# agstub/shakti-fenics

Hardware: NVIDIA B200
Metric: time_steps_per_sec_at_16M_dofs (higher is better)
Workload: dtype f64

## Files before the change

shakti-fenics_b200/csrc/amg.cu:

```cuda
#include "amg.h"
#include "comm.h"

#include <algorithm>
#include <cstdlib>
#include <cmath>
#include <map>
#include <numeric>

namespace shakti {


static int aggregate(const HostCsr& A, int32_t n, const std::vector<uint8_t>& excl, const std::vector<uint8_t>& strong,
                     std::vector<int32_t>& agg) {
  agg.assign(n, -1);
  std::vector<uint8_t> free_(n, 1);
  for (int32_t i = 0; i < n; ++i)
    if (!excl.empty() && excl[i]) free_[i] = 0;
  int32_t na = 0;
  auto nb = [&](int32_t i, auto&& f) {
    for (int32_t k = A.rowptr[i]; k < A.rowptr[i + 1]; ++k) {
      const int32_t j = A.col[k];
      if (j < n && j != i && (excl.empty() || !excl[j]) && (strong.empty() || strong[k])) f(j);
    }
  };
  for (int32_t i = 0; i < n; ++i) {
    if (!free_[i]) continue;
    bool ok = true;
    nb(i, [&](int32_t j) { ok &= (free_[j] != 0); });
    if (!ok) continue;
    agg[i] = na;
    free_[i] = 0;
    nb(i, [&](int32_t j) { agg[j] = na; free_[j] = 0; });
    ++na;
  }
  {
    std::vector<int32_t> snap(agg);
    std::vector<int32_t> size(na, 0);
    for (int32_t i = 0; i < n; ++i)
      if (snap[i] >= 0) size[snap[i]]++;
    for (int32_t i = 0; i < n; ++i) {
      if (!free_[i]) continue;
      int32_t best = -1;
      nb(i, [&](int32_t j) {
        if (snap[j] >= 0 && (best < 0 || size[snap[j]] < size[best])) best = snap[j];
      });
      if (best >= 0) { agg[i] = best; size[best]++; free_[i] = 0; }
    }
  }
  for (int32_t i = 0; i < n; ++i) {
    if (!free_[i]) continue;
    agg[i] = na;
    free_[i] = 0;
    nb(i, [&](int32_t j) { if (free_[j]) { agg[j] = na; free_[j] = 0; } });
    ++na;
  }
  return na;
}

static HostCsr product_pattern(const HostCsr& A, const HostCsr& B) {
  HostCsr C;
  C.n_rows = A.n_rows;
  C.n_cols = B.n_cols;
  C.rowptr.assign(A.n_rows + 1, 0);
  std::vector<int32_t> mark(B.n_cols, -1), tmp;
  for (int64_t i = 0; i < A.n_rows; ++i) {
    tmp.clear();
    for (int32_t k = A.rowptr[i]; k < A.rowptr[i + 1]; ++k) {
      const int32_t j = A.col[k];
      if (j >= B.n_rows) continue;
      for (int32_t l = B.rowptr[j]; l < B.rowptr[j + 1]; ++l) {
        const int32_t c = B.col[l];
        if (mark[c] != (int32_t)i) { mark[c] = (int32_t)i; tmp.push_back(c); }
      }
    }
    std::sort(tmp.begin(), tmp.end());
    C.col.insert(C.col.end(), tmp.begin(), tmp.end());
    if (C.col.size() > 2000000000ULL) throw Error(SHAKTI_ERR_INVALID, "AMG product pattern too large");
    C.rowptr[i + 1] = (int32_t)C.col.size();
  }
  return C;
}


__global__ void amg_dinv_kernel(int32_t n, const int32_t* __restrict__ diag_pos, const double* __restrict__ val,
                                double* __restrict__ dinv) {
  const int32_t i = blockIdx.x * blockDim.x + threadIdx.x;
  if (i >= n) return;
  const double d = val[diag_pos[i]];
  dinv[i] = d != 0.0 ? 1.0 / d : 0.0;
}

__global__ void __launch_bounds__(256)
amg_prolongator_kernel(SellView A, const uint8_t* __restrict__ pmap, const int32_t* __restrict__ diag_pos,
                       const double* __restrict__ dinv, double omega, const int32_t* __restrict__ Pslice,
                       double* __restrict__ Pval) {
  const int32_t row = blockIdx.x * blockDim.x + threadIdx.x;
  if (row >= A.n_rows) return;
  const int32_t slice = row >> 5, lane = row & 31;
  const int32_t base = A.slice_ptr[slice];
  const int32_t w = (A.slice_ptr[slice + 1] - base) >> 5;
  const int32_t pbase = Pslice[slice] + lane;
  const int32_t dpos = diag_pos[row];
  const double s = omega * dinv[row];
  for (int k = 0; k < w; ++k) {
    const int32_t p = base + 32 * k + lane;
    const uint8_t t = pmap[p];
    if (t == 255) continue;
    const double v = (p == dpos ? 1.0 : 0.0) - s * A.val[p];
    Pval[pbase + 32 * (int32_t)t] += v;
  }
}

__global__ void amg_gather_vals_kernel(int64_t n, const int32_t* __restrict__ map, const double* __restrict__ src,
                                       double* __restrict__ out) {
  const int64_t stride = (int64_t)gridDim.x * blockDim.x;
  for (int64_t i = (int64_t)blockIdx.x * blockDim.x + threadIdx.x; i < n; i += stride) {
    const int32_t m = map[i];
    out[i] = m >= 0 ? src[m] : 0.0;
  }
}

__global__ void __launch_bounds__(128)
amg_spgemm_kernel(SellView A, const int32_t* __restrict__ Alen, SellView B, const int32_t* __restrict__ Blen,
                  int32_t Bn_rows, const int32_t* __restrict__ Cslice, const int32_t* __restrict__ Ccol,
                  const int32_t* __restrict__ Clen, double* __restrict__ Cval) {
  const int32_t row = blockIdx.x * blockDim.x + threadIdx.x;
  if (row >= A.n_rows) return;
  const int32_t lane = row & 31;
  const int32_t abase = A.slice_ptr[row >> 5] + lane;
  const int32_t cbase = Cslice[row >> 5] + lane;
  const int32_t clen = Clen[row];
  const int32_t alen = Alen[row];
  for (int ka = 0; ka < alen; ++ka) {
    const int32_t j = A.col[abase + 32 * ka];
    if (j >= Bn_rows) continue;
    const double a = A.val[abase + 32 * ka];
    if (a == 0.0) continue;
    const int32_t bbase = B.slice_ptr[j >> 5] + (j & 31);
    const int32_t blen = Blen[j];
    for (int kb = 0; kb < blen; ++kb) {
      const int32_t c = B.col[bbase + 32 * kb];
      const double b = B.val[bbase + 32 * kb];
      int lo = 0, hi = clen - 1;
      while (lo < hi) {
        const int mid = (lo + hi) >> 1;
        if (Ccol[cbase + 32 * mid] < c) lo = mid + 1; else hi = mid;
      }
      Cval[cbase + 32 * lo] += a * b;
    }
  }
}

__global__ void __launch_bounds__(128)
amg_spgemm_warp_kernel(SellView A, const int32_t* __restrict__ Alen, SellView B, const int32_t* __restrict__ Blen,
                       int32_t Bn_rows, const int32_t* __restrict__ Cslice, const int32_t* __restrict__ Ccol,
                       const int32_t* __restrict__ Clen, double* __restrict__ Cval) {
  const int32_t row = (blockIdx.x * blockDim.x + threadIdx.x) >> 5;
  const int lane = threadIdx.x & 31;
  if (row >= A.n_rows) return;
  const int32_t abase = A.slice_ptr[row >> 5] + (row & 31);
  const int32_t cbase = Cslice[row >> 5] + (row & 31);
  const int32_t clen = Clen[row], alen = Alen[row];
  for (int pos = lane; pos < clen; pos += 32) {
    const int32_t c = Ccol[cbase + 32 * pos];
    double acc = 0.0;
    for (int ka = 0; ka < alen; ++ka) {
      const int32_t j = A.col[abase + 32 * ka];
      if (j >= Bn_rows) continue;
      const double a = A.val[abase + 32 * ka];
      if (a == 0.0) continue;
      const int32_t bbase = B.slice_ptr[j >> 5] + (j & 31);
      int lo = 0, hi = Blen[j] - 1;
      while (lo < hi) {
        const int mid = (lo + hi) >> 1;
        if (B.col[bbase + 32 * mid] < c) lo = mid + 1; else hi = mid;
      }
      if (hi >= 0 && lo == hi && B.col[bbase + 32 * lo] == c) acc += a * B.val[bbase + 32 * lo];
    }
    Cval[cbase + 32 * pos] = acc;
  }
}

struct SpgemmPlan {
  bool built = false, ok = false;
  DevBuf<int64_t> prod_ptr;
  DevBuf<uint8_t> slot;
};

__global__ void __launch_bounds__(128)
amg_spgemm_count_kernel(SellView A, const int32_t* __restrict__ Alen, const int32_t* __restrict__ Blen, int32_t Bn_rows,
                        int32_t* __restrict__ slice_width) {
  const int32_t row = blockIdx.x * blockDim.x + threadIdx.x;
  int32_t cnt = 0;
  if (row < A.n_rows) {
    const int32_t abase = A.slice_ptr[row >> 5] + (row & 31);
    const int32_t alen = Alen[row];
    for (int ka = 0; ka < alen; ++ka) {
      const int32_t j = A.col[abase + 32 * ka];
      if (j < Bn_rows) cnt += Blen[j];
    }
  }
#pragma unroll
  for (int o = 16; o > 0; o >>= 1) cnt = max(cnt, __shfl_xor_sync(0xffffffffu, cnt, o));
  if ((threadIdx.x & 31) == 0 && (row >> 5) < A.n_slices) slice_width[row >> 5] = cnt;
}

__global__ void __launch_bounds__(128)
amg_spgemm_slots_kernel(SellView A, const int32_t* __restrict__ Alen, SellView B, const int32_t* __restrict__ Blen,
                        int32_t Bn_rows, const int32_t* __restrict__ Cslice, const int32_t* __restrict__ Ccol,
                        const int32_t* __restrict__ Clen, const int64_t* __restrict__ prod_ptr, uint8_t* __restrict__ slot) {
  const int32_t row = blockIdx.x * blockDim.x + threadIdx.x;
  if (row >= A.n_rows) return;
  const int32_t lane = row & 31;
  const int32_t abase = A.slice_ptr[row >> 5] + lane;
  const int32_t cbase = Cslice[row >> 5] + lane;
  const int32_t clen = Clen[row], alen = Alen[row];
  uint8_t* __restrict__ sp = slot + prod_ptr[row >> 5] + lane;
  int64_t t = 0;
  for (int ka = 0; ka < alen; ++ka) {
    const int32_t j = A.col[abase + 32 * ka];
    if (j >= Bn_rows) continue;
    const int32_t bbase = B.slice_ptr[j >> 5] + (j & 31);
    const int32_t blen = Blen[j];
    for (int kb = 0; kb < blen; ++kb, ++t) {
      const int32_t c = B.col[bbase + 32 * kb];
      int lo = 0, hi = clen - 1;
      while (lo < hi) {
        const int mid = (lo + hi) >> 1;
        if (Ccol[cbase + 32 * mid] < c) lo = mid + 1; else hi = mid;
      }
      sp[32 * t] = (uint8_t)lo;
    }
  }
}

__global__ void __launch_bounds__(128)
amg_spgemm_table_kernel(SellView A, const int32_t* __restrict__ Alen, SellView B, const int32_t* __restrict__ Blen,
                        int32_t Bn_rows, const int32_t* __restrict__ Cslice, const int32_t* __restrict__ Clen,
                        const int64_t* __restrict__ prod_ptr, const uint8_t* __restrict__ slot, double* __restrict__ Cval) {
  extern __shared__ double acc[];
  const int32_t row = blockIdx.x * blockDim.x + threadIdx.x;
  if (row >= A.n_rows) return;
  const int32_t lane = row & 31;
  const int32_t abase = A.slice_ptr[row >> 5] + lane;
  const int32_t clen = Clen[row], alen = Alen[row];
  double* __restrict__ my = acc + threadIdx.x;
  for (int k = 0; k < clen; ++k) my[k * 128] = 0.0;
  const uint8_t* __restrict__ sp = slot + prod_ptr[row >> 5] + lane;
  int64_t t = 0;
  for (int ka = 0; ka < alen; ++ka) {
    const int32_t j = A.col[abase + 32 * ka];
    if (j >= Bn_rows) continue;
    const double a = A.val[abase + 32 * ka];
    const int32_t bbase = B.slice_ptr[j >> 5] + (j & 31);
    const int32_t blen = Blen[j];
    for (int kb = 0; kb < blen; ++kb, ++t) my[(int)sp[32 * t] * 128] += a * B.val[bbase + 32 * kb];
  }
  double* __restrict__ cp = Cval + Cslice[row >> 5] + lane;
  for (int k = 0; k < clen; ++k) cp[32 * k] = my[k * 128];
}

static void build_spgemm_plan(const DevSell& A, const DevSell& B, const DevSell& C, SpgemmPlan& plan, cudaStream_t s) {
  plan.built = true;
  plan.ok = false;
  const size_t smem = (size_t)C.max_width * 128 * sizeof(double);
  if (A.n_rows == 0 || C.max_width > 255 || smem > 96 * 1024) return;
  DevBuf<int32_t> width;
  width.alloc_zero(A.n_slices, s);
  SHAKTI_LAUNCH(amg_spgemm_count_kernel, div_up((int64_t)A.n_slices * 32, 128), 128, 0, s, view(A), A.rowlen.p, B.rowlen.p, B.n_rows,
                width.p);
  const std::vector<int32_t> w = width.download(s);
  std::vector<int64_t> ptr(w.size() + 1, 0);
  for (size_t i = 0; i < w.size(); ++i) ptr[i + 1] = ptr[i] + 32 * (int64_t)w[i];
  plan.prod_ptr.upload(ptr);
  plan.slot.alloc((size_t)std::max<int64_t>(ptr.back(), 1));
  SHAKTI_LAUNCH(amg_spgemm_slots_kernel, div_up(A.n_rows, 128), 128, 0, s, view(A), A.rowlen.p, view(B), B.rowlen.p, B.n_rows,
                C.slice_ptr.p, C.col.p, C.rowlen.p, plan.prod_ptr.p, plan.slot.p);
  if (smem > 48 * 1024)
    SHAKTI_CUDA(cudaFuncSetAttribute(amg_spgemm_table_kernel, cudaFuncAttributeMaxDynamicSharedMemorySize, 96 * 1024));
  plan.ok = true;
}

static void spgemm_numeric(const DevSell& A, const DevSell& B, DevSell& C, SpgemmPlan& plan, cudaStream_t s) {
  if (A.n_rows == 0) return;
  if (A.n_rows <= 400000) {
    SHAKTI_LAUNCH(amg_spgemm_warp_kernel, div_up((int64_t)A.n_rows * 32, 128), 128, 0, s, view(A), A.rowlen.p, view(B), B.rowlen.p,
                  B.n_rows, C.slice_ptr.p, C.col.p, C.rowlen.p, C.val.p);
    return;
  }
  if (!plan.built) build_spgemm_plan(A, B, C, plan, s);
  if (plan.ok) {
    SHAKTI_LAUNCH(amg_spgemm_table_kernel, div_up(A.n_rows, 128), 128, (size_t)C.max_width * 128 * sizeof(double), s, view(A),
                  A.rowlen.p, view(B), B.rowlen.p, B.n_rows, C.slice_ptr.p, C.rowlen.p, plan.prod_ptr.p, plan.slot.p, C.val.p);
  } else {
    SHAKTI_CUDA(cudaMemsetAsync(C.val.p, 0, sizeof(double) * C.padded, s));
    SHAKTI_LAUNCH(amg_spgemm_kernel, div_up(A.n_rows, 128), 128, 0, s, view(A), A.rowlen.p, view(B), B.rowlen.p, B.n_rows,
                  C.slice_ptr.p, C.col.p, C.rowlen.p, C.val.p);
  }
}

__global__ void amg_dense_fill_kernel(SellView A, const int32_t* __restrict__ Alen, int32_t n, double* __restrict__ D) {
  const int32_t row = blockIdx.x * blockDim.x + threadIdx.x;
  if (row >= n) return;
  const int32_t base = A.slice_ptr[row >> 5] + (row & 31);
  for (int k = 0; k < Alen[row]; ++k) {
    const int32_t j = A.col[base + 32 * k];
    if (j < n) D[(size_t)row * 2 * n + j] += A.val[base + 32 * k];
  }
  D[(size_t)row * 2 * n + n + row] = 1.0;
}

__global__ void __launch_bounds__(1024)
amg_dense_invert_kernel(int32_t n, double* __restrict__ D, int* __restrict__ info) {
  extern __shared__ double fcol[];
  __shared__ int piv;
  __shared__ double pval;
  const int ld = 2 * n;
  for (int k = 0; k < n; ++k) {
    if (threadIdx.x < 32) {
      int p = k;
      double best = -1.0;
      for (int i = k + (int)threadIdx.x; i < n; i += 32) {
        const double v = fabs(D[(size_t)i * ld + k]);
        if (v > best) { best = v; p = i; }
      }
#pragma unroll
      for (int o = 16; o > 0; o >>= 1) {
        const double ob = __shfl_xor_sync(0xffffffffu, best, o);
        const int op = __shfl_xor_sync(0xffffffffu, p, o);
        if (ob > best || (ob == best && op < p)) { best = ob; p = op; }
      }
      if (threadIdx.x == 0) {
        piv = p;
        pval = D[(size_t)p * ld + k];
        if (!(best > 0.0)) *info = k + 1;
      }
    }
    __syncthreads();
    const int p = piv;
    const double inv = pval != 0.0 ? 1.0 / pval : 0.0;
    for (int j = threadIdx.x; j < ld; j += blockDim.x) {
      const double a = D[(size_t)p * ld + j], b = D[(size_t)k * ld + j];
      D[(size_t)p * ld + j] = b;
      D[(size_t)k * ld + j] = a * inv;
    }
    __syncthreads();
    for (int i = threadIdx.x; i < n; i += blockDim.x) fcol[i] = (i == k) ? 0.0 : D[(size_t)i * ld + k];
    __syncthreads();
    for (int idx = threadIdx.x; idx < n * ld; idx += blockDim.x) {
      const int i = idx / ld, j = idx - i * ld;
      const double f = fcol[i];
      if (f != 0.0) D[(size_t)i * ld + j] -= f * D[(size_t)k * ld + j];
    }
    __syncthreads();
  }
}

template <class TB, class TX>
__global__ void amg_dense_apply_kernel(int32_t n, const double* __restrict__ D, const TB* __restrict__ b,
                                       TX* __restrict__ x) {
  pdl_sync();
  const int warp = (blockIdx.x * blockDim.x + threadIdx.x) >> 5, lane = threadIdx.x & 31;
  if (warp >= n) return;
  const double* row = D + (size_t)warp * 2 * n + n;
  double acc = 0.0;
  for (int j = lane; j < n; j += 32) acc += row[j] * (double)b[j];
#pragma unroll
  for (int o = 16; o > 0; o >>= 1) acc += __shfl_xor_sync(0xffffffffu, acc, o);
  if (lane == 0) x[warp] = (TX)acc;
}

template <class T, int KG>
__global__ void __launch_bounds__(256)
amg_cheby_kernel(SellViewT<T> A, const T* __restrict__ dinv, const T* __restrict__ b, const T* __restrict__ x,
                 T* __restrict__ d, T* __restrict__ x_out, T c1, T c2) {
  pdl_sync();
  int32_t row;
  T acc = 0;
  if (KG == 1) {
    row = blockIdx.x * blockDim.x + threadIdx.x;
    const int32_t slice = row >> 5;
    if (slice >= A.n_slices) return;
    const int32_t base = A.slice_ptr[slice];
    const int32_t w = (A.slice_ptr[slice + 1] - base) >> 5;
    const int32_t* __restrict__ cp = A.col + base + (row & 31);
    const T* __restrict__ vp = A.val + base + (row & 31);
#pragma unroll 4
    for (int k = 0; k < w; ++k) acc += vp[32 * k] * x[cp[32 * k]];
  } else {
    __shared__ T psum[KG][32];
    const int32_t slice = blockIdx.x;
    const int lane = threadIdx.x & 31, g = threadIdx.x >> 5;
    row = slice * 32 + lane;
    const int32_t base = A.slice_ptr[slice];
    const int32_t w = (A.slice_ptr[slice + 1] - base) >> 5;
    const int32_t* __restrict__ cp = A.col + base + lane;
    const T* __restrict__ vp = A.val + base + lane;
    for (int k = g; k < w; k += KG) acc += vp[32 * k] * x[cp[32 * k]];
    psum[g][lane] = acc;
    __syncthreads();
    if (g != 0) return;
#pragma unroll
    for (int j = 1; j < KG; ++j) acc += psum[j][lane];
  }
  if (row >= A.n_rows) return;
  const T r = dinv[row] * (b[row] - acc);
  const T dn = c1 * d[row] + c2 * r;
  d[row] = dn;
  x_out[row] = x[row] + dn;
}
constexpr int32_t kChebyWideRowsBelow = 300000;
template <class T>
static void launch_cheby(SellViewT<T> A, const T* dinv, const T* b, const T* x, T* d, T* x_out, double c1, double c2, cudaStream_t s) {
  if (A.n_rows < kChebyWideRowsBelow)
    SHAKTI_LAUNCH_PDL((amg_cheby_kernel<T, 8>), A.n_slices, 256, 0, s, A, dinv, b, x, d, x_out, (T)c1, (T)c2);
  else
    SHAKTI_LAUNCH_PDL((amg_cheby_kernel<T, 1>), div_up((int64_t)A.n_slices * 32, 256), 256, 0, s, A, dinv, b, x, d, x_out, (T)c1, (T)c2);
}

__global__ void __launch_bounds__(256)
amg_cheby_h_kernel(int32_t n_rows, int32_t n_slices, const int32_t* __restrict__ slice_ptr, const int32_t* __restrict__ col,
                   const __half* __restrict__ val, const float* __restrict__ dinv, const float* __restrict__ b,
                   const float* __restrict__ x, float* __restrict__ d, float* __restrict__ x_out, float c1, float c2) {
  pdl_sync();
  const int32_t row = blockIdx.x * blockDim.x + threadIdx.x;
  const int32_t slice = row >> 5;
  if (slice >= n_slices) return;
  const int32_t base = slice_ptr[slice];
  const int32_t w = (slice_ptr[slice + 1] - base) >> 5;
  const int32_t* __restrict__ cp = col + base + (row & 31);
  const __half* __restrict__ vp = val + base + (row & 31);
  float acc = 0.f;
#pragma unroll 4
  for (int k = 0; k < w; ++k) acc += __half2float(vp[32 * k]) * x[cp[32 * k]];
  if (row >= n_rows) return;
  const float r = dinv[row] * b[row] - acc;
  const float dn = c1 * d[row] + c2 * r;
  d[row] = dn;
  x_out[row] = x[row] + dn;
}
__global__ void __launch_bounds__(256)
amg_resid_h_kernel(int32_t n_rows, int32_t n_slices, const int32_t* __restrict__ slice_ptr, const int32_t* __restrict__ col,
                   const __half* __restrict__ val, const float* __restrict__ dinv, const float* __restrict__ b,
                   const float* __restrict__ x, float* __restrict__ r) {
  pdl_sync();
  const int32_t row = blockIdx.x * blockDim.x + threadIdx.x;
  const int32_t slice = row >> 5;
  if (slice >= n_slices) return;
  const int32_t base = slice_ptr[slice];
  const int32_t w = (slice_ptr[slice + 1] - base) >> 5;
  const int32_t* __restrict__ cp = col + base + (row & 31);
  const __half* __restrict__ vp = val + base + (row & 31);
  float acc = 0.f;
#pragma unroll 4
  for (int k = 0; k < w; ++k) acc += __half2float(vp[32 * k]) * x[cp[32 * k]];
  if (row >= n_rows) return;
  const float di = dinv[row];
  r[row] = b[row] - (di != 0.f ? acc / di : 0.f);
}
static bool uses_half(const Amg::Impl& I, const DevSell& A);

template <class T>
__global__ void amg_cheby_first_kernel(int32_t n, const T* __restrict__ dinv, const T* __restrict__ b, T inv_theta,
                                       T* __restrict__ d, T* __restrict__ x) {
  pdl_sync();
  const int32_t i = blockIdx.x * blockDim.x + threadIdx.x;
  if (i >= n) return;
  const T v = dinv[i] * b[i] * inv_theta;
  d[i] = v;
  x[i] = v;
}

__global__ void __launch_bounds__(256)
amg_gershgorin_kernel(SellView A, const double* __restrict__ dinv, unsigned long long* __restrict__ out) {
  const int32_t row = blockIdx.x * blockDim.x + threadIdx.x;
  double v = 0.0;
  if (row < A.n_rows) {
    const int32_t base = A.slice_ptr[row >> 5] + (row & 31);
    const int32_t w = (A.slice_ptr[(row >> 5) + 1] - A.slice_ptr[row >> 5]) >> 5;
    double acc = 0.0;
    for (int k = 0; k < w; ++k) acc += fabs(A.val[base + 32 * k]);
    v = fabs(dinv[row]) * acc;
  }
#pragma unroll
  for (int o = 16; o > 0; o >>= 1) v = fmax(v, __shfl_xor_sync(0xffffffffu, v, o));
  if ((threadIdx.x & 31) == 0 && v > 0.0) atomicMax(out, (unsigned long long)__double_as_longlong(v));
}

__global__ void amg_pack_rows_kernel(int64_t n, const int32_t* __restrict__ pos, const double* __restrict__ val,
                                     double* __restrict__ out) {
  const int64_t i = (int64_t)blockIdx.x * blockDim.x + threadIdx.x;
  if (i >= n) return;
  const int32_t p = pos[i];
  out[i] = p >= 0 ? val[p] : 0.0;
}
__global__ void amg_unpack_rows_kernel(int64_t n, const int32_t* __restrict__ pos, const double* __restrict__ in,
                                       double* __restrict__ val) {
  const int64_t i = (int64_t)blockIdx.x * blockDim.x + threadIdx.x;
  if (i >= n) return;
  const int32_t p = pos[i];
  if (p >= 0) val[p] = in[i];
}
__global__ void amg_dense_rows_kernel(SellView A, const int32_t* __restrict__ Alen, const int32_t* __restrict__ colmap,
                                      int32_t n, int32_t N, double* __restrict__ D) {
  const int32_t row = blockIdx.x * blockDim.x + threadIdx.x;
  if (row >= n) return;
  const int32_t base = A.slice_ptr[row >> 5] + (row & 31);
  for (int k = 0; k < Alen[row]; ++k) D[(size_t)row * N + colmap[A.col[base + 32 * k]]] += A.val[base + 32 * k];
}
__global__ void amg_dense_assemble_kernel(int32_t N, int32_t nmax, int32_t nranks, const int32_t* __restrict__ off,
                                          const double* __restrict__ G, double* __restrict__ D) {
  const int64_t t = (int64_t)blockIdx.x * blockDim.x + threadIdx.x;
  if (t >= (int64_t)N * N) return;
  const int32_t gi = (int32_t)(t / N), j = (int32_t)(t - (int64_t)gi * N);
  int r = 0;
  while (r + 1 < nranks && off[r + 1] <= gi) ++r;
  const int32_t li = gi - off[r];
  D[(size_t)gi * 2 * N + j] = G[((size_t)r * nmax + li) * N + j];
  if (j == 0) D[(size_t)gi * 2 * N + N + gi] = 1.0;
}
template <class TO>
__global__ void amg_compact_kernel(int32_t N, int32_t nmax, int32_t nranks, const int32_t* __restrict__ off,
                                   const double* __restrict__ G, TO* __restrict__ out) {
  const int32_t gi = blockIdx.x * blockDim.x + threadIdx.x;
  if (gi >= N) return;
  int r = 0;
  while (r + 1 < nranks && off[r + 1] <= gi) ++r;
  out[gi] = (TO)G[(size_t)r * nmax + (gi - off[r])];
}

template <class T>
__global__ void amg_gather_map_kernel(int32_t n, const int32_t* __restrict__ map, const T* __restrict__ src, T* __restrict__ out) {
  pdl_sync();
  const int32_t i = blockIdx.x * blockDim.x + threadIdx.x;
  if (i < n) out[i] = src[map[i]];
}

template <class TI, class TO>
__global__ void amg_convert_kernel(int32_t n, const TI* __restrict__ in, TO* __restrict__ out) {
  const int32_t i = blockIdx.x * blockDim.x + threadIdx.x;
  if (i < n) out[i] = (TO)in[i];
}

template <class T>
struct CycleVecs {
  DevBuf<T> x, x2, b, r, d, dinv;
};

struct AmgLevel {
  int32_t n = 0, n_ghost = 0, n_cols = 0;
  int32_t n_coarse = 0, n_coarse_ghost = 0;
  int64_t nnz = 0;
  DevSell A;
  DevBuf<int32_t> diag_pos;
  DevBuf<double> dinv;
  DevSell P, R, AP;
  SpgemmPlan plan_AP, plan_RAP;
  DevBuf<uint8_t> pmap;
  DevBuf<int32_t> tmap;
  CycleVecs<double> vd;
  CycleVecs<float> vf;
  double lmax = 2.0;
  bool last = false;
  HostCsr hA;
  HostSell hS;
  std::vector<Neighbor> nbrs;
  HaloPlan own_halo;
  HaloPlan* halo = nullptr;
  int maxw = 0;
  DevBuf<int32_t> psend_pos, pg_pos;
  DevBuf<double> psend, precv;
};

struct Amg::Impl {
  AmgOptions opt;
  cudaStream_t s = 0;
  const HostCsr* A0 = nullptr;
  const HostSell* S0 = nullptr;
  const std::vector<Neighbor>* nbrs0 = nullptr;
  HaloPlan* halo0 = nullptr;
  std::vector<uint8_t> exclude;
  std::vector<std::unique_ptr<AmgLevel>> lv;
  DevBuf<double> dense, dense_rows, dense_gather, crhs, cgather, cglob, csol;
  DevBuf<int32_t> coff, ccolmap;
  int32_t cN = 0, cnmax = 0, coff_me = 0;
  DevBuf<int> info;
  bool dense_coarse = false;
  bool built = false;
  double op_complexity = 0.0;
  Reducer red;
  DevBuf<double> scal, lmax_dev;
  double* host_scal = nullptr;
  cudaGraphExec_t gexec = nullptr;
  bool graph_valid = false;
  bool warm = false;
  int64_t graph_launches = 0;
  void* result_ptr = nullptr;
  int tail_level = -1;
  std::unique_ptr<Amg> tail;
  HostCsr tailA;
  HostSell tailS;
  DevSell tailM;
  DevBuf<int32_t> tail_diag;
  int32_t tail_N = 0, tail_nmax = 0, tail_wmax = 0;
  DevBuf<int32_t> tail_pack_pos;
  DevBuf<int32_t> tail_unpack_pos;
  DevBuf<double> tail_send, tail_recv;
  DevBuf<int32_t> tail_gid;
  DevBuf<int32_t> tail_off;
  HaloPlan tail_halo;
  std::vector<Neighbor> no_nbrs;
  int sm_count = 148;
  P2pGather tail_gather;
  DevBuf<double> tail_rhs_d, tail_gather_d;
  ~Impl() {
    if (host_scal) cudaFreeHost(host_scal);
    if (gexec) cudaGraphExecDestroy(gexec);
  }
};

Amg::Amg() : p_(new Impl()) {}
Amg::~Amg() = default;
int Amg::levels() const { return (int)p_->lv.size() + (p_->tail ? p_->tail->levels() - 1 : 0); }
bool Amg::fp32() const { return p_->opt.fp32_cycle != 0; }
double Amg::operator_complexity() const { return p_->op_complexity; }

static std::vector<int32_t> diag_positions(const HostCsr& A, const HostSell& S, int32_t n) {
  std::vector<int32_t> d(n, 0);
  for (int32_t r = 0; r < n; ++r) {
    const int32_t* b = A.col.data() + A.rowptr[r];
    const int32_t* e = A.col.data() + A.rowptr[r + 1];
    const int32_t* p = std::lower_bound(b, e, r);
    if (p == e || *p != r) throw Error(SHAKTI_ERR_INVALID, "AMG: matrix row without diagonal entry");
    d[r] = (int32_t)S.pos(r, (int)(p - b));
  }
  return d;
}

void Amg::setup(const HostCsr& A0, const HostSell& S0, const std::vector<uint8_t>& exclude, const std::vector<Neighbor>& nbrs,
                HaloPlan* halo, const AmgOptions& opt, int sm_count, cudaStream_t s) {
  Impl& I = *p_;
  I.opt = opt;
  I.s = s;
  I.A0 = &A0;
  I.S0 = &S0;
  I.nbrs0 = &nbrs;
  I.halo0 = halo;
  I.exclude = exclude;
  I.lv.clear();
  I.built = false;
  I.graph_valid = false;
  I.warm = false;
  I.red.init(sm_count);
  I.sm_count = sm_count;
  I.tail.reset();
  I.tail_level = -1;
  I.scal.alloc_zero(4, s);
  if (!I.host_scal) SHAKTI_CUDA(cudaMallocHost(&I.host_scal, 32 * sizeof(double)));
  refreshes_ = 0;
}

template <class T>
static void alloc_cycle_vectors(CycleVecs<T>& v, const AmgLevel& L, cudaStream_t s) {
  v.x.alloc_zero(std::max(L.n_cols, 1), s);
  v.x2.alloc_zero(std::max(L.n_cols, 1), s);
  v.b.alloc_zero(std::max(L.n, 1), s);
  v.r.alloc_zero(std::max(L.n, 1), s);
  v.d.alloc_zero(std::max(L.n, 1), s);
  v.dinv.alloc_zero(std::max(L.n, 1), s);
}
static void alloc_level_vectors(AmgLevel& L, bool fp32, cudaStream_t s) {
  L.dinv.alloc_zero(std::max(L.n, 1), s);
  if (fp32) alloc_cycle_vectors(L.vf, L, s);
  else alloc_cycle_vectors(L.vd, L, s);
}
template <class T> static CycleVecs<T>& vecs(AmgLevel& L);
template <> CycleVecs<double>& vecs<double>(AmgLevel& L) { return L.vd; }
template <> CycleVecs<float>& vecs<float>(AmgLevel& L) { return L.vf; }

static void numeric_level(Amg::Impl& I, size_t l, const DevSell& Afine, const int32_t* fine_diag_pos) {
  cudaStream_t s = I.s;
  AmgLevel& L = *I.lv[l];
  const DevSell& A = (l == 0) ? Afine : L.A;
  const int32_t* dpos = (l == 0) ? fine_diag_pos : L.diag_pos.p;
  if (L.n > 0) SHAKTI_LAUNCH(amg_dinv_kernel, div_up(L.n, 256), 256, 0, s, L.n, dpos, A.val.p, L.dinv.p);
  if (L.last) return;
  SHAKTI_CUDA(cudaMemsetAsync(L.P.val.p, 0, sizeof(double) * L.P.padded, s));
  if (L.n > 0)
    SHAKTI_LAUNCH(amg_prolongator_kernel, div_up(L.n, 256), 256, 0, s, view(A), L.pmap.p, dpos, L.dinv.p,
                  I.opt.prolong_omega, L.P.slice_ptr.p, L.P.val.p);
  if (comm().active() && L.maxw > 0) {
    const int64_t ns = (int64_t)L.halo->n_send_total() * L.maxw, ng = (int64_t)L.n_ghost * L.maxw;
    if (ns) SHAKTI_LAUNCH(amg_pack_rows_kernel, div_up(ns, 256), 256, 0, s, ns, L.psend_pos.p, L.P.val.p, L.psend.p);
    L.halo->exchange_packed(L.psend.p, L.precv.p, L.n, L.maxw, s);
    if (ng) SHAKTI_LAUNCH(amg_unpack_rows_kernel, div_up(ng, 256), 256, 0, s, ng, L.pg_pos.p, L.precv.p, L.P.val.p);
  }
  if (L.R.padded)
    SHAKTI_LAUNCH(amg_gather_vals_kernel, (int)std::min<int64_t>(148 * 8, std::max<int64_t>(1, (L.R.padded + 255) / 256)), 256, 0, s,
                  L.R.padded, L.tmap.p, L.P.val.p, L.R.val.p);
  spgemm_numeric(A, L.P, L.AP, L.plan_AP, s);
  spgemm_numeric(L.R, L.AP, I.lv[l + 1]->A, L.plan_RAP, s);
}

static bool uses_half(const Amg::Impl& I, const DevSell& A) {
  static const bool on = getenv("SHAKTI_AMG_FP16") != nullptr && atoi(getenv("SHAKTI_AMG_FP16")) != 0;
  return on && I.opt.fp32_cycle && I.opt.smoother == 1 && A.n_rows >= kChebyWideRowsBelow;
}

static void sync_cycle_precision(Amg::Impl& I, size_t l, const DevSell& Afine, bool matrices) {
  cudaStream_t s = I.s;
  AmgLevel& L = *I.lv[l];
  const DevSell& A = (l == 0) ? Afine : L.A;
  if (I.opt.fp32_cycle) {
    launch_d2f(L.n, L.dinv.p, L.vf.dinv.p, s);
    if (uses_half(I, A)) A.refresh_f16_scaled(L.dinv.p, s);
    else A.refresh_f32(s);
    if (matrices && !L.last) { L.P.refresh_f32(s); L.R.refresh_f32(s); }
  } else if (L.n) {
    SHAKTI_CUDA(cudaMemcpyAsync(L.vd.dinv.p, L.dinv.p, sizeof(double) * L.n, cudaMemcpyDeviceToDevice, s));
  }
}

static void update_smoother_bounds(Amg::Impl& I, const DevSell& Afine) {
  cudaStream_t s = I.s;
  const size_t nl = I.lv.size();
  if (I.opt.smoother != 1) return;
  if (I.lmax_dev.n < nl) { I.lmax_dev.alloc_zero(std::max<size_t>(nl, 16), s); }
  SHAKTI_CUDA(cudaMemsetAsync(I.lmax_dev.p, 0, sizeof(double) * nl, s));
  for (size_t l = 0; l < nl; ++l) {
    AmgLevel& L = *I.lv[l];
    if (L.n > 0)
      SHAKTI_LAUNCH(amg_gershgorin_kernel, div_up(L.n, 256), 256, 0, s, view(l == 0 ? Afine : L.A), L.dinv.p,
                    reinterpret_cast<unsigned long long*>(I.lmax_dev.p + l));
  }
  comm_allreduce_max(I.lmax_dev.p, (int)nl, s);
  std::vector<double> h(nl);
  SHAKTI_REQUIRE(nl <= 32, "AMG: more than 32 levels");
  launch_readback(I.lmax_dev.p, I.host_scal, (int)nl, s);
  SHAKTI_CUDA(cudaStreamSynchronize(s));
  for (size_t l = 0; l < nl; ++l) h[l] = I.host_scal[l];
  for (size_t l = 0; l < nl; ++l) I.lv[l]->lmax = (h[l] > 0 && std::isfinite(h[l])) ? h[l] : 2.0;
}

static void coarsen_level(Amg::Impl& I, size_t l, const DevSell& dA, const HostCsr& A, const HostSell& S,
                          const std::vector<uint8_t>& excl, bool& stalled) {
  cudaStream_t s = I.s;
  const AmgOptions& opt = I.opt;
  AmgLevel& L = *I.lv[l];
  const int me = comm().rank, nranks = comm().nranks;
  const int32_t n = L.n, g = L.n_ghost;
  std::vector<uint8_t> strong;
  const double theta = opt.strength_theta * std::pow(0.5, (double)l);
  if (theta > 0 && n > 0) {
    std::vector<double> v = dA.val.download(s);
    std::vector<double> diag(n, 0.0);
    for (int32_t i = 0; i < n; ++i)
      for (int32_t k = A.rowptr[i]; k < A.rowptr[i + 1]; ++k)
        if (A.col[k] == i) diag[i] = std::fabs(v[S.pos(i, k - A.rowptr[i])]);
    strong.assign(A.nnz(), 0);
    for (int32_t i = 0; i < n; ++i)
      for (int32_t k = A.rowptr[i]; k < A.rowptr[i + 1]; ++k) {
        const int32_t j = A.col[k];
        if (j >= n || j == i) continue;
        const double a = std::fabs(v[S.pos(i, k - A.rowptr[i])]);
        strong[k] = (a >= theta * std::sqrt(diag[i] * diag[j])) && a > 0;
      }
  }
  std::vector<int32_t> agg;
  const int32_t nc = n > 0 ? aggregate(A, n, excl, strong, agg) : 0;
  const double nc_glob = comm_host_sum((double)nc, s), n_glob = comm_host_sum((double)n, s);
  if (nc_glob <= 0 || nc_glob > 0.85 * n_glob) { stalled = true; return; }
  stalled = false;
  L.n_coarse = nc;
  std::vector<int> gowner(g, -1);
  for (const auto& nb : L.nbrs)
    for (int32_t k = 0; k < nb.recv_count; ++k) gowner[nb.recv_begin - n + k] = nb.rank;
  std::vector<double> gagg(g, -1.0);
  if (comm().active()) {
    std::vector<double> tmp((size_t)n + g, -1.0);
    for (int32_t i = 0; i < n; ++i) tmp[i] = (double)agg[i];
    DevBuf<double> dv;
    dv.upload(tmp);
    L.halo->exchange(dv.p, s);
    tmp = dv.download(s);
    for (int32_t k = 0; k < g; ++k) gagg[k] = tmp[n + k];
  }
  typedef std::pair<int, int32_t> Gid;
  auto gid_of_col = [&](int32_t j) -> Gid {
    if (j < n) return agg[j] >= 0 ? Gid(me, agg[j]) : Gid(-1, -1);
    const double a = gagg[j - n];
    return a >= 0 ? Gid(gowner[j - n], (int32_t)a) : Gid(-1, -1);
  };
  const bool smoothed = opt.prolong_omega != 0.0;
  std::vector<std::vector<Gid>> prow((size_t)n + g);
  for (int32_t i = 0; i < n; ++i) {
    if (agg[i] < 0) continue;
    auto& r = prow[i];
    if (smoothed) {
      for (int32_t k = A.rowptr[i]; k < A.rowptr[i + 1]; ++k) {
        const Gid c = gid_of_col(A.col[k]);
        if (c.first >= 0) r.push_back(c);
      }
      std::sort(r.begin(), r.end());
      r.erase(std::unique(r.begin(), r.end()), r.end());
    } else {
      r.push_back(Gid(me, agg[i]));
    }
  }
  int maxw = 0;
  const std::vector<int32_t>& sidx = L.halo->send_idx_host;
  for (int32_t v : sidx) maxw = std::max<int>(maxw, (int)prow[v].size());
  maxw = (int)comm_host_max((double)maxw, s);
  L.maxw = comm().active() ? maxw : 0;
  if (comm().active() && maxw > 0) {
    const int wp = 1 + 2 * maxw;
    std::vector<double> sb((size_t)std::max<size_t>(sidx.size(), 1) * wp, -1.0), rb((size_t)std::max(g, 1) * wp, -1.0);
    for (size_t k = 0; k < sidx.size(); ++k) {
      const auto& r = prow[sidx[k]];
      sb[k * wp] = (double)r.size();
      for (size_t w = 0; w < r.size(); ++w) { sb[k * wp + 1 + 2 * w] = r[w].first; sb[k * wp + 2 + 2 * w] = r[w].second; }
    }
    DevBuf<double> dsb, drb;
    dsb.upload(sb);
    drb.upload(rb);
    L.halo->exchange_packed(dsb.p, drb.p, n, wp, s);
    rb = drb.download(s);
    for (int32_t k = 0; k < g; ++k) {
      const int len = (int)rb[(size_t)k * wp];
      for (int w = 0; w < len; ++w)
        prow[(size_t)n + k].push_back(Gid((int)rb[(size_t)k * wp + 1 + 2 * w], (int32_t)rb[(size_t)k * wp + 2 + 2 * w]));
    }
  }
  std::vector<Gid> gset;
  for (const auto& r : prow)
    for (const Gid& c : r)
      if (c.first != me) gset.push_back(c);
  std::sort(gset.begin(), gset.end());
  gset.erase(std::unique(gset.begin(), gset.end()), gset.end());
  const int32_t gc = (int32_t)gset.size();
  L.n_coarse_ghost = gc;
  auto local_col = [&](const Gid& c) -> int32_t {
    if (c.first == me) return c.second;
    return nc + (int32_t)(std::lower_bound(gset.begin(), gset.end(), c) - gset.begin());
  };
  HostCsr P;
  P.n_rows = (int64_t)n + g;
  P.n_cols = (int64_t)nc + gc;
  P.rowptr.assign(P.n_rows + 1, 0);
  std::vector<std::vector<int32_t>> order((size_t)g);
  {
    std::vector<std::pair<int32_t, int>> tmp;
    for (int64_t i = 0; i < P.n_rows; ++i) {
      tmp.clear();
      for (size_t w = 0; w < prow[i].size(); ++w) tmp.push_back({local_col(prow[i][w]), (int)w});
      std::sort(tmp.begin(), tmp.end());
      if (i >= n) order[i - n].assign(tmp.size(), 0);
      for (size_t q = 0; q < tmp.size(); ++q) {
        P.col.push_back(tmp[q].first);
        if (i >= n) order[i - n][tmp[q].second] = (int32_t)q;
      }
      P.rowptr[i + 1] = (int32_t)P.col.size();
    }
  }
  HostSell PS = sell_from_csr(P);
  {
    std::vector<uint8_t> pm(S.padded(), 255);
    for (int32_t i = 0; i < n; ++i) {
      const int32_t* pb = P.col.data() + P.rowptr[i];
      const int32_t* pe = P.col.data() + P.rowptr[i + 1];
      if (pb == pe) continue;
      for (int32_t k = A.rowptr[i]; k < A.rowptr[i + 1]; ++k) {
        const int32_t j = A.col[k];
        if (!smoothed && j != i) continue;
        const Gid c = gid_of_col(j);
        if (c.first < 0) continue;
        const int32_t* q = std::lower_bound(pb, pe, local_col(c));
        const int64_t t = q - pb;
        if (t > 254) throw Error(SHAKTI_ERR_INVALID, "AMG: prolongator row too long");
        pm[S.pos(i, k - A.rowptr[i])] = (uint8_t)t;
      }
    }
    L.pmap.upload(pm);
  }
  L.P.upload_pattern(PS, P.nnz());
  if (L.maxw > 0) {
    std::vector<int32_t> sp((size_t)std::max<size_t>(sidx.size(), 1) * L.maxw, -1), gp((size_t)std::max(g, 1) * L.maxw, -1);
    for (size_t k = 0; k < sidx.size(); ++k) {
      const int32_t i = sidx[k];
      const int32_t* pb = P.col.data() + P.rowptr[i];
      const int32_t* pe = P.col.data() + P.rowptr[i + 1];
      for (size_t w = 0; w < prow[i].size(); ++w) {
        const int32_t* q = std::lower_bound(pb, pe, local_col(prow[i][w]));
        sp[k * L.maxw + w] = (int32_t)PS.pos(i, (int)(q - pb));
      }
    }
    for (int32_t k = 0; k < g; ++k)
      for (size_t w = 0; w < order[k].size(); ++w) gp[(size_t)k * L.maxw + w] = (int32_t)PS.pos((int64_t)n + k, order[k][w]);
    L.psend_pos.upload(sp);
    L.pg_pos.upload(gp);
    L.psend.alloc_zero(sp.size(), s);
    L.precv.alloc_zero(gp.size(), s);
  }
  HostCsr Pown;
  Pown.n_rows = n;
  Pown.n_cols = nc;
  Pown.rowptr.assign((size_t)n + 1, 0);
  std::vector<int32_t> pown_entry;
  for (int32_t i = 0; i < n; ++i) {
    for (int32_t k = P.rowptr[i]; k < P.rowptr[i + 1]; ++k)
      if (P.col[k] < nc) { Pown.col.push_back(P.col[k]); pown_entry.push_back(k); }
    Pown.rowptr[i + 1] = (int32_t)Pown.col.size();
  }
  std::vector<int32_t> tentry;
  HostCsr R = csr_transpose(Pown, &tentry);
  HostSell RS = sell_from_csr(R);
  {
    std::vector<int32_t> ppos = sell_positions(P, PS);
    std::vector<int32_t> tm(RS.padded(), -1);
    for (int64_t r = 0; r < R.n_rows; ++r)
      for (int32_t k = R.rowptr[r]; k < R.rowptr[r + 1]; ++k) tm[RS.pos(r, k - R.rowptr[r])] = ppos[pown_entry[tentry[k]]];
    L.tmap.upload(tm);
  }
  L.R.upload_pattern(RS, R.nnz());
  HostCsr AP = product_pattern(A, P);
  L.AP.upload_pattern(sell_from_csr(AP), AP.nnz());
  std::unique_ptr<AmgLevel> Ln(new AmgLevel());
  Ln->hA = product_pattern(R, AP);
  Ln->hA.n_cols = (int64_t)nc + gc;
  Ln->hS = sell_from_csr(Ln->hA);
  Ln->n = nc;
  Ln->n_ghost = gc;
  Ln->n_cols = nc + gc;
  Ln->nnz = Ln->hA.nnz();
  Ln->A.upload_pattern(Ln->hS, Ln->hA.nnz());
  Ln->diag_pos.upload(diag_positions(Ln->hA, Ln->hS, nc));
  if (comm().active()) {
    std::vector<std::vector<double>> ask(nranks);
    std::vector<int32_t> rb(nranks, 0), rc(nranks, 0);
    for (int32_t k = 0; k < gc; ++k) {
      const int o = gset[k].first;
      if (rc[o] == 0) rb[o] = nc + k;
      rc[o]++;
      ask[o].push_back((double)gset[k].second);
    }
    std::vector<std::vector<double>> asked = comm_exchange_lists(ask, s);
    for (int r = 0; r < nranks; ++r) {
      if (r == me || (asked[r].empty() && rc[r] == 0)) continue;
      Neighbor nb;
      nb.rank = r;
      for (double v : asked[r]) nb.send_local.push_back((int32_t)v);
      nb.recv_begin = rb[r];
      nb.recv_count = rc[r];
      Ln->nbrs.push_back(std::move(nb));
    }
  }
  Ln->own_halo.build(Ln->nbrs);
  Ln->halo = &Ln->own_halo;
  alloc_level_vectors(*Ln, I.opt.fp32_cycle != 0, s);
  I.lv.push_back(std::move(Ln));
}

static void build_tail(Amg::Impl& I, size_t l) {
  cudaStream_t s = I.s;
  AmgLevel& L = *I.lv[l];
  const HostCsr& A = (l == 0) ? *I.A0 : L.hA;
  const HostSell& S = (l == 0) ? *I.S0 : L.hS;
  const int me = comm().rank, nr = comm().nranks;
  const int32_t n = L.n;
  const std::vector<double> counts = comm_host_allgather((double)n, s);
  std::vector<int32_t> off(nr + 1, 0), cnt(nr, 0);
  int32_t nmax = 1;
  for (int r = 0; r < nr; ++r) {
    cnt[r] = (int32_t)counts[r];
    off[r + 1] = off[r] + cnt[r];
    nmax = std::max(nmax, cnt[r]);
  }
  const int32_t N = off[nr];
  std::vector<int32_t> gid(std::max(L.n_cols, 1), 0);
  {
    std::vector<double> tmp((size_t)std::max(L.n_cols, 1), 0.0);
    for (int32_t c = 0; c < n; ++c) tmp[c] = (double)(off[me] + c);
    DevBuf<double> dv;
    dv.upload(tmp);
    L.halo->exchange(dv.p, s);
    tmp = dv.download(s);
    for (int32_t c = 0; c < L.n_cols; ++c) gid[c] = (int32_t)tmp[c];
  }
  int32_t wloc = 1;
  for (int32_t i = 0; i < n; ++i) wloc = std::max(wloc, A.rowptr[i + 1] - A.rowptr[i]);
  const int32_t wmax = (int32_t)comm_host_max((double)wloc, s);
  std::vector<double> mine;
  mine.reserve((size_t)n + A.nnz());
  for (int32_t i = 0; i < n; ++i) {
    mine.push_back((double)(A.rowptr[i + 1] - A.rowptr[i]));
    for (int32_t k = A.rowptr[i]; k < A.rowptr[i + 1]; ++k) mine.push_back((double)gid[A.col[k]]);
  }
  const std::vector<std::vector<double>> in = comm_exchange_lists(std::vector<std::vector<double>>(nr, mine), s);
  HostCsr& G = I.tailA;
  G = HostCsr();
  G.n_rows = G.n_cols = N;
  G.rowptr.assign((size_t)N + 1, 0);
  std::vector<int32_t> order;
  std::vector<std::pair<int32_t, int32_t>> tmp;
  for (int r = 0; r < nr; ++r) {
    const std::vector<double>& v = in[r];
    size_t p = 0;
    for (int32_t i = 0; i < cnt[r]; ++i) {
      const int len = (int)v[p++];
      tmp.clear();
      for (int k = 0; k < len; ++k) tmp.push_back({(int32_t)v[p++], k});
      std::sort(tmp.begin(), tmp.end());
      const size_t base = order.size();
      order.resize(base + len);
      for (int q = 0; q < len; ++q) {
        G.col.push_back(tmp[q].first);
        order[base + tmp[q].second] = q;
      }
      G.rowptr[(size_t)off[r] + i + 1] = (int32_t)G.col.size();
    }
  }
  I.tailS = sell_from_csr(G);
  std::vector<int32_t> unpack((size_t)nr * nmax * wmax, -1), pack((size_t)nmax * wmax, -1);
  {
    size_t e = 0;
    for (int r = 0; r < nr; ++r)
      for (int32_t i = 0; i < cnt[r]; ++i) {
        const int32_t gr = off[r] + i;
        const int len = G.rowptr[gr + 1] - G.rowptr[gr];
        for (int k = 0; k < len; ++k, ++e) unpack[((size_t)r * nmax + i) * wmax + k] = (int32_t)I.tailS.pos(gr, order[e]);
      }
  }
  for (int32_t i = 0; i < n; ++i)
    for (int32_t k = A.rowptr[i]; k < A.rowptr[i + 1]; ++k) pack[(size_t)i * wmax + (k - A.rowptr[i])] = (int32_t)S.pos(i, k - A.rowptr[i]);
  I.tail_N = N; I.tail_nmax = nmax; I.tail_wmax = wmax;
  I.tail_pack_pos.upload(pack);
  I.tail_unpack_pos.upload(unpack);
  I.tail_send.alloc_zero((size_t)nmax * wmax, s);
  I.tail_recv.alloc_zero((size_t)nr * nmax * wmax, s);
  I.tail_gid.upload(gid);
  I.tail_off.upload(off);
  I.tailM.upload_pattern(I.tailS, G.nnz());
  I.tail_diag.upload(diag_positions(G, I.tailS, N));
  if (comm().p2p) {
    I.tail_gather.build(nmax, s);
    I.tail_gather.set_counts(cnt);
  } else {
    I.tail_rhs_d.alloc_zero(nmax, s);
    I.tail_gather_d.alloc_zero((size_t)nr * nmax, s);
  }
  AmgOptions to = I.opt;
  to.cuda_graph = 0;
  I.tail.reset(new Amg());
  I.tail_level = (int)l;
  {
    CommSerialScope serial;
    I.tail->setup(I.tailA, I.tailS, std::vector<uint8_t>(), I.no_nbrs, &I.tail_halo, to, I.sm_count, s);
  }
}

static void refresh_tail(Amg::Impl& I, const DevSell& Afine) {
  if (!I.tail) return;
  cudaStream_t s = I.s;
  const DevSell& A = (I.tail_level == 0) ? Afine : I.lv[I.tail_level]->A;
  const int64_t blk = (int64_t)I.tail_nmax * I.tail_wmax;
  SHAKTI_LAUNCH(amg_pack_rows_kernel, div_up(blk, 256), 256, 0, s, blk, I.tail_pack_pos.p, A.val.p, I.tail_send.p);
  comm_allgather(I.tail_send.p, I.tail_recv.p, (int)blk, s);
  const int64_t tot = blk * comm().nranks;
  SHAKTI_LAUNCH(amg_unpack_rows_kernel, div_up(tot, 256), 256, 0, s, tot, I.tail_unpack_pos.p, I.tail_recv.p, I.tailM.val.p);
  CommSerialScope serial;
  I.tail->refresh(I.tailM, I.tail_diag.p);
}

static void build_hierarchy(Amg::Impl& I, const DevSell& Afine, const int32_t* fine_diag_pos) {
  cudaStream_t s = I.s;
  const AmgOptions& opt = I.opt;
  I.lv.clear();
  {
    std::unique_ptr<AmgLevel> L0(new AmgLevel());
    L0->n = (int32_t)I.A0->n_rows;
    L0->n_cols = (int32_t)I.A0->n_cols;
    L0->n_ghost = L0->n_cols - L0->n;
    L0->nnz = I.A0->nnz();
    L0->nbrs = *I.nbrs0;
    L0->halo = I.halo0;
    alloc_level_vectors(*L0, I.opt.fp32_cycle != 0, s);
    I.lv.push_back(std::move(L0));
  }
  std::vector<uint8_t> excl = I.exclude;
  double nnz_sum = 0.0;
  for (size_t l = 0;; ++l) {
    AmgLevel& L = *I.lv[l];
    const HostCsr& A = (l == 0) ? *I.A0 : L.hA;
    const HostSell& S = (l == 0) ? *I.S0 : L.hS;
    const DevSell& dA = (l == 0) ? Afine : L.A;
    nnz_sum += (double)A.nnz();
    const double n_glob = comm_host_sum((double)L.n, s);
    bool stop = (n_glob <= opt.coarse_size) || ((int)l + 1 >= opt.max_levels);
    if (comm().active() && n_glob <= std::max(opt.replicate_below, opt.coarse_size)) {
      build_tail(I, l);
      L.last = true;
      numeric_level(I, l, Afine, fine_diag_pos);
      break;
    }
    bool stalled = false;
    if (!stop) coarsen_level(I, l, dA, A, S, excl, stalled);
    if (stop || stalled) {
      if (comm().active() && n_glob <= 4.0e6) build_tail(I, l);
      L.last = true;
      numeric_level(I, l, Afine, fine_diag_pos);
      break;
    }
    numeric_level(I, l, Afine, fine_diag_pos);
    excl.clear();
  }
  AmgLevel& last = *I.lv.back();
  const std::vector<double> counts = comm_host_allgather((double)last.n, s);
  int64_t N = 0, nmax = 0;
  std::vector<int32_t> off(counts.size() + 1, 0);
  for (size_t r = 0; r < counts.size(); ++r) {
    off[r + 1] = off[r] + (int32_t)counts[r];
    nmax = std::max<int64_t>(nmax, (int64_t)counts[r]);
  }
  N = off.back();
  I.dense_coarse = N <= 1024 && N > 0 && !I.tail;
  if (I.dense_coarse) {
    const int me = comm().rank, nr = comm().nranks;
    I.cN = (int32_t)N;
    I.cnmax = (int32_t)nmax;
    I.coff_me = off[me];
    I.coff.upload(off);
    std::vector<int32_t> colmap(std::max(last.n_cols, 1), 0);
    for (int32_t c = 0; c < last.n; ++c) colmap[c] = off[me] + c;
    if (last.n_ghost > 0) {
      std::vector<double> tmp((size_t)last.n_cols, 0.0);
      for (int32_t c = 0; c < last.n; ++c) tmp[c] = (double)(off[me] + c);
      DevBuf<double> dv;
      dv.upload(tmp);
      last.halo->exchange(dv.p, s);
      tmp = dv.download(s);
      for (int32_t c = last.n; c < last.n_cols; ++c) colmap[c] = (int32_t)tmp[c];
    }
    I.ccolmap.upload(colmap);
    I.dense.alloc_zero((size_t)2 * N * N, s);
    I.dense_rows.alloc_zero((size_t)std::max<int64_t>(nmax, 1) * N, s);
    I.dense_gather.alloc_zero((size_t)nr * std::max<int64_t>(nmax, 1) * N, s);
    I.crhs.alloc_zero(std::max<int64_t>(nmax, 1), s);
    I.cgather.alloc_zero((size_t)nr * std::max<int64_t>(nmax, 1), s);
    I.cglob.alloc_zero(N, s);
    I.csol.alloc_zero(N, s);
    I.info.alloc_zero(1, s);
  }
  const double nnz0 = comm_host_sum((double)I.A0->nnz(), s);
  nnz_sum = comm_host_sum(nnz_sum, s);
  I.op_complexity = nnz0 > 0 ? nnz_sum / nnz0 : 0.0;
  I.built = true;
  if (I.tail) {
    refresh_tail(I, Afine);
    const double nnz_root = (double)I.tailA.nnz();
    if (nnz0 > 0) I.op_complexity += (I.tail->operator_complexity() - 1.0) * nnz_root / nnz0;
  }
}

void Amg::refresh_fine_smoother(const DevSell& Afine, const int32_t* fine_diag_pos) {
  Impl& I = *p_;
  cudaStream_t s = I.s;
  if (!I.built || I.lv.empty()) return;
  I.graph_valid = false;
  AmgLevel& L = *I.lv[0];
  if (L.n > 0) SHAKTI_LAUNCH(amg_dinv_kernel, div_up(L.n, 256), 256, 0, s, L.n, fine_diag_pos, Afine.val.p, L.dinv.p);
  if (I.opt.smoother != 1 || (L.last && I.dense_coarse)) { sync_cycle_precision(I, 0, Afine, false); return; }
  SHAKTI_CUDA(cudaMemsetAsync(I.scal.p + 1, 0, sizeof(double), s));
  if (L.n > 0)
    SHAKTI_LAUNCH(amg_gershgorin_kernel, div_up(L.n, 256), 256, 0, s, view(Afine), L.dinv.p,
                  reinterpret_cast<unsigned long long*>(I.scal.p + 1));
  comm_allreduce_max(I.scal.p + 1, 1, s);
  launch_readback(I.scal.p + 1, I.host_scal, 1, s);
  SHAKTI_CUDA(cudaStreamSynchronize(s));
  if (I.host_scal[0] > 0 && std::isfinite(I.host_scal[0])) L.lmax = I.host_scal[0];
  sync_cycle_precision(I, 0, Afine, false);
}

void Amg::refresh(const DevSell& Afine, const int32_t* fine_diag_pos) {
  Impl& I = *p_;
  cudaStream_t s = I.s;
  I.graph_valid = false;
  if (!I.built) { build_hierarchy(I, Afine, fine_diag_pos); I.warm = false; }
  else {
    { SHAKTI_PHASE("rf_numeric", s); for (size_t l = 0; l < I.lv.size(); ++l) numeric_level(I, l, Afine, fine_diag_pos); }
    { SHAKTI_PHASE("rf_tail", s); refresh_tail(I, Afine); }
  }
  { SHAKTI_PHASE("rf_bounds", s); update_smoother_bounds(I, Afine); }
  { SHAKTI_PHASE("rf_f32", s); for (size_t l = 0; l < I.lv.size(); ++l) sync_cycle_precision(I, l, Afine, true); }
  if (I.dense_coarse) {
    AmgLevel& L = *I.lv.back();
    const DevSell& A = (I.lv.size() == 1) ? Afine : L.A;
    const int32_t N = I.cN, nmax = std::max(I.cnmax, 1);
    SHAKTI_CUDA(cudaMemsetAsync(I.dense_rows.p, 0, sizeof(double) * (size_t)nmax * N, s));
    if (L.n > 0)
      SHAKTI_LAUNCH(amg_dense_rows_kernel, div_up(L.n, 128), 128, 0, s, view(A), A.rowlen.p, I.ccolmap.p, L.n, N, I.dense_rows.p);
    comm_allgather(I.dense_rows.p, I.dense_gather.p, nmax * N, s);
    SHAKTI_CUDA(cudaMemsetAsync(I.dense.p, 0, sizeof(double) * 2 * (size_t)N * N, s));
    SHAKTI_CUDA(cudaMemsetAsync(I.info.p, 0, sizeof(int), s));
    SHAKTI_LAUNCH(amg_dense_assemble_kernel, div_up((int64_t)N * N, 256), 256, 0, s, N, nmax, comm().nranks, I.coff.p,
                  I.dense_gather.p, I.dense.p);
    SHAKTI_LAUNCH(amg_dense_invert_kernel, 1, 1024, N * sizeof(double), s, N, I.dense.p, I.info.p);
  }
  ++refreshes_;
}

template <class T>
static void cheby_step(Amg::Impl& I, const DevSell& A, const T* dinv, const T* b, const T* x, T* d, T* x_out, double c1, double c2,
                       cudaStream_t s) {
  launch_cheby<T>(view_as<T>(A), dinv, b, x, d, x_out, c1, c2, s);
}
template <>
void cheby_step<float>(Amg::Impl& I, const DevSell& A, const float* dinv, const float* b, const float* x, float* d, float* x_out,
                       double c1, double c2, cudaStream_t s) {
  if (uses_half(I, A))
    SHAKTI_LAUNCH_PDL(amg_cheby_h_kernel, div_up((int64_t)A.n_slices * 32, 256), 256, 0, s, A.n_rows, A.n_slices, A.slice_ptr.p, A.col.p,
                      A.valh.p, dinv, b, x, d, x_out, (float)c1, (float)c2);
  else
    launch_cheby<float>(viewf(A), dinv, b, x, d, x_out, c1, c2, s);
}
template <class T>
static void level_residual(Amg::Impl& I, const DevSell& A, const T* dinv, const T* x, const T* b, T* r, cudaStream_t s) {
  launch_residual<T>(view_as<T>(A), x, b, r, s);
}
template <>
void level_residual<float>(Amg::Impl& I, const DevSell& A, const float* dinv, const float* x, const float* b, float* r, cudaStream_t s) {
  if (uses_half(I, A))
    SHAKTI_LAUNCH_PDL(amg_resid_h_kernel, div_up((int64_t)A.n_slices * 32, 256), 256, 0, s, A.n_rows, A.n_slices, A.slice_ptr.p, A.col.p,
                      A.valh.p, dinv, b, x, r);
  else
    launch_residual<float>(viewf(A), x, b, r, s);
}

template <class T>
static void smooth(Amg::Impl& I, AmgLevel& L, const DevSell& A, const T* b, int sweeps, bool zero_guess, bool ghosts_current) {
  cudaStream_t s = I.s;
  CycleVecs<T>& v = vecs<T>(L);
  if (sweeps <= 0) {
    if (zero_guess) launch_fill_t<T>(L.n, (T)0, v.x.p, s);
    return;
  }
  if (I.opt.smoother == 1) {
    const double hi = L.lmax, lo = L.lmax / I.opt.cheby_ratio;
    const double theta = 0.5 * (hi + lo), delta = 0.5 * (hi - lo), sigma = theta / delta;
    double rho = 1.0 / sigma;
    int k0 = 0;
    if (zero_guess) {
      if (L.n) SHAKTI_LAUNCH_PDL((amg_cheby_first_kernel<T>), div_up(L.n, 256), 256, 0, s, L.n, v.dinv.p, b, (T)(1.0 / theta), v.d.p, v.x.p);
      k0 = 1;
    }
    for (int k = k0; k < sweeps; ++k) {
      double c1, c2;
      if (k == 0) { c1 = 0.0; c2 = 1.0 / theta; }
      else {
        const double rho_n = 1.0 / (2.0 * sigma - rho);
        c1 = rho_n * rho;
        c2 = 2.0 * rho_n / delta;
        rho = rho_n;
      }
      if (I.opt.smoother_halo && !(ghosts_current && k == k0)) L.halo->exchange(v.x.p, s);
      if (L.n) cheby_step<T>(I, A, v.dinv.p, b, v.x.p, v.d.p, v.x2.p, c1, c2, s);
      std::swap(v.x.p, v.x2.p);
    }
  } else {
    const double om = I.opt.smoother_omega;
    int k0 = 0;
    if (zero_guess) { launch_scaled_mul<T>(L.n, v.dinv.p, b, om, v.x.p, s); k0 = 1; }
    for (int k = k0; k < sweeps; ++k) {
      if (I.opt.smoother_halo && !(ghosts_current && k == k0)) L.halo->exchange(v.x.p, s);
      launch_jacobi<T>(view_as<T>(A), v.dinv.p, b, v.x.p, v.x2.p, om, s);
      std::swap(v.x.p, v.x2.p);
    }
  }
}

template <class T>
static void vcycle(Amg::Impl& I, const DevSell& Afine) {
  cudaStream_t s = I.s;
  const int nl = (int)I.lv.size();
  for (int l = 0; l < nl; ++l) {
    AmgLevel& L = *I.lv[l];
    CycleVecs<T>& v = vecs<T>(L);
    const DevSell& A = (l == 0) ? Afine : L.A;
    if (l == I.tail_level) {
      T* tb = I.tail->rhs_buffer<T>();
      if (comm().p2p) {
        I.tail_gather.allgatherv<T, T>(v.b.p, tb, s);
      } else {
        SHAKTI_CUDA(cudaMemsetAsync(I.tail_rhs_d.p, 0, sizeof(double) * I.tail_nmax, s));
        if (L.n) SHAKTI_LAUNCH((amg_convert_kernel<T, double>), div_up(L.n, 256), 256, 0, s, L.n, v.b.p, I.tail_rhs_d.p);
        comm_allgather(I.tail_rhs_d.p, I.tail_gather_d.p, I.tail_nmax, s);
        SHAKTI_LAUNCH((amg_compact_kernel<T>), div_up(I.tail_N, 128), 128, 0, s, I.tail_N, I.tail_nmax, comm().nranks, I.tail_off.p,
                      I.tail_gather_d.p, tb);
      }
      const T* tx;
      {
        CommSerialScope serial;
        tx = I.tail->cycle<T>(I.tailM);
      }
      if (L.n_cols) SHAKTI_LAUNCH_PDL((amg_gather_map_kernel<T>), div_up(L.n_cols, 256), 256, 0, s, L.n_cols, I.tail_gid.p, tx, v.x.p);
      break;
    }
    if (L.last) {
      if (I.dense_coarse) {
        const int32_t N = I.cN, nmax = std::max(I.cnmax, 1);
        if (comm().active()) {
          SHAKTI_CUDA(cudaMemsetAsync(I.crhs.p, 0, sizeof(double) * nmax, s));
          if (L.n) SHAKTI_LAUNCH((amg_convert_kernel<T, double>), div_up(L.n, 256), 256, 0, s, L.n, v.b.p, I.crhs.p);
          comm_allgather(I.crhs.p, I.cgather.p, nmax, s);
          SHAKTI_LAUNCH((amg_compact_kernel<double>), div_up(N, 128), 128, 0, s, N, nmax, comm().nranks, I.coff.p, I.cgather.p, I.cglob.p);
          SHAKTI_LAUNCH((amg_dense_apply_kernel<double, double>), div_up((int64_t)N * 32, 128), 128, 0, s, N, I.dense.p, I.cglob.p, I.csol.p);
          if (L.n) SHAKTI_LAUNCH((amg_convert_kernel<double, T>), div_up(L.n, 256), 256, 0, s, L.n, I.csol.p + I.coff_me, v.x.p);
        } else if (L.n) {
          SHAKTI_LAUNCH_PDL((amg_dense_apply_kernel<T, T>), div_up((int64_t)L.n * 32, 128), 128, 0, s, L.n, I.dense.p, v.b.p, v.x.p);
        }
      } else {
        smooth<T>(I, L, A, v.b.p, 8, true, false);
      }
      break;
    }
    smooth<T>(I, L, A, v.b.p, I.opt.presmooth, true, false);
    L.halo->exchange(v.x.p, s);
    level_residual<T>(I, A, v.dinv.p, v.x.p, v.b.p, v.r.p, s);
    launch_spmv<T>(view_as<T>(L.R), v.r.p, vecs<T>(*I.lv[l + 1]).b.p, s);
  }
  for (int l = nl - 2; l >= 0; --l) {
    AmgLevel& L = *I.lv[l];
    CycleVecs<T>& v = vecs<T>(L);
    const DevSell& A = (l == 0) ? Afine : L.A;
    AmgLevel& C = *I.lv[l + 1];
    if (l + 1 != I.tail_level) C.halo->exchange(vecs<T>(C).x.p, s);
    launch_spmv_add<T>(view_as<T>(L.P), vecs<T>(C).x.p, v.x.p, s);
    smooth<T>(I, L, A, v.b.p, I.opt.postsmooth, false, true);
  }
}

template <class T>
static void run_cycle(Amg::Impl& I, const DevSell& Afine) {
  cudaStream_t s = I.s;
  std::vector<std::pair<T*, T*>> saved;
  for (auto& L : I.lv) saved.push_back({vecs<T>(*L).x.p, vecs<T>(*L).x2.p});
  auto restore = [&]() {
    I.result_ptr = vecs<T>(*I.lv[0]).x.p;
    for (size_t l = 0; l < I.lv.size(); ++l) { vecs<T>(*I.lv[l]).x.p = saved[l].first; vecs<T>(*I.lv[l]).x2.p = saved[l].second; }
  };
  if (!I.opt.cuda_graph || !I.warm) {
    vcycle<T>(I, Afine);
    restore();
    I.warm = true;
    return;
  }
  if (!I.graph_valid) {
    const int64_t before = g_kernel_launches;
    SHAKTI_CUDA(cudaStreamBeginCapture(s, cudaStreamCaptureModeRelaxed));
    cudaGraph_t graph = nullptr;
    try {
      vcycle<T>(I, Afine);
    } catch (...) {
      cudaStreamEndCapture(s, &graph);
      if (graph) cudaGraphDestroy(graph);
      restore();
      throw;
    }
    SHAKTI_CUDA(cudaStreamEndCapture(s, &graph));
    restore();
    I.graph_launches = g_kernel_launches - before;
    g_kernel_launches = before;
    bool updated = false;
    if (I.gexec) {
      cudaGraphExecUpdateResultInfo info;
      updated = cudaGraphExecUpdate(I.gexec, graph, &info) == cudaSuccess;
      if (!updated) { cudaGetLastError(); cudaGraphExecDestroy(I.gexec); I.gexec = nullptr; }
    }
    if (!updated) SHAKTI_CUDA(cudaGraphInstantiate(&I.gexec, graph, 0));
    SHAKTI_CUDA(cudaGraphDestroy(graph));
    I.graph_valid = true;
  }
  SHAKTI_CUDA(cudaGraphLaunch(I.gexec, s));
  g_kernel_launches += I.graph_launches;
}

bool Amg::launch_level_smoother(int level, const DevSell& Afine, int64_t* rows, int64_t* nnz, int* value_bytes) {
  Impl& I = *p_;
  if (!I.built || level < 0 || level >= (int)I.lv.size()) return false;
  AmgLevel& L = *I.lv[level];
  const DevSell& A = (level == 0) ? Afine : L.A;
  if (rows) *rows = L.n;
  if (nnz) *nnz = A.nnz;
  if (value_bytes) *value_bytes = uses_half(I, A) ? 2 : (I.opt.fp32_cycle ? 4 : 8);
  if (L.n == 0) return true;
  if (I.opt.fp32_cycle) cheby_step<float>(I, A, L.vf.dinv.p, L.vf.b.p, L.vf.x.p, L.vf.d.p, L.vf.x2.p, 0.3, 0.2, I.s);
  else launch_cheby<double>(view(A), L.vd.dinv.p, L.vd.b.p, L.vd.x.p, L.vd.d.p, L.vd.x2.p, 0.3, 0.2, I.s);
  return true;
}

template <class T> T* Amg::rhs_buffer() { return vecs<T>(*p_->lv[0]).b.p; }
template <class T> const T* Amg::cycle(const DevSell& Afine) {
  run_cycle<T>(*p_, Afine);
  return static_cast<const T*>(p_->result_ptr);
}
template float* Amg::rhs_buffer<float>();
template double* Amg::rhs_buffer<double>();
template const float* Amg::cycle<float>(const DevSell&);
template const double* Amg::cycle<double>(const DevSell&);

void Amg::apply(const DevSell& Afine, const double* rin, double* z) {
  Impl& I = *p_;
  cudaStream_t s = I.s;
  AmgLevel& L0 = *I.lv[0];
  if (I.opt.fp32_cycle) {
    launch_d2f(L0.n, rin, L0.vf.b.p, s);
    run_cycle<float>(I, Afine);
    launch_f2d(L0.n, static_cast<const float*>(I.result_ptr), z, s);
  } else {
    if (L0.n) SHAKTI_CUDA(cudaMemcpyAsync(L0.vd.b.p, rin, sizeof(double) * L0.n, cudaMemcpyDeviceToDevice, s));
    run_cycle<double>(I, Afine);
    if (L0.n) SHAKTI_CUDA(cudaMemcpyAsync(z, I.result_ptr, sizeof(double) * L0.n, cudaMemcpyDeviceToDevice, s));
  }
}

}

extern "C" int shakti_host_amg_aggregate(int32_t n, const int32_t* rowptr, const int32_t* col, const double* val,
                                         double theta, const uint8_t* exclude, int32_t* agg_out, int32_t* n_agg) {
  try {
    if (n <= 0 || !rowptr || !col || !agg_out || !n_agg) throw shakti::Error(SHAKTI_ERR_INVALID, "bad arguments");
    shakti::HostCsr A;
    A.n_rows = A.n_cols = n;
    A.rowptr.assign(rowptr, rowptr + n + 1);
    A.col.assign(col, col + rowptr[n]);
    std::vector<uint8_t> excl;
    if (exclude) excl.assign(exclude, exclude + n);
    std::vector<uint8_t> strong;
    if (theta > 0 && val) {
      std::vector<double> diag(n, 0.0);
      for (int32_t i = 0; i < n; ++i)
        for (int32_t k = rowptr[i]; k < rowptr[i + 1]; ++k)
          if (col[k] == i) diag[i] = std::fabs(val[k]);
      strong.assign(A.nnz(), 0);
      for (int32_t i = 0; i < n; ++i)
        for (int32_t k = rowptr[i]; k < rowptr[i + 1]; ++k) {
          const int32_t j = col[k];
          if (j == i) continue;
          const double a = std::fabs(val[k]);
          strong[k] = (a >= theta * std::sqrt(diag[i] * diag[j])) && a > 0;
        }
    }
    std::vector<int32_t> agg;
    *n_agg = shakti::aggregate(A, n, excl, strong, agg);
    std::copy(agg.begin(), agg.end(), agg_out);
    return SHAKTI_OK;
  } catch (const std::exception& e) {
    shakti::set_last_error(e.what());
    return SHAKTI_ERR_INVALID;
  }
}
```

shakti-fenics_b200/csrc/device.h:

```cpp
#pragma once
#include <cuda_fp16.h>

#include "common.h"
#include "prep.h"

namespace shakti {

struct DevParams {
  double g, rho_i, rho_w, nu, Lh, omega, n, A;
  double cm;
  double rwg;
  double inv_rwg, inv_Lh, cm_over_Lh;
  int n_is_3;
};

DevParams make_dev_params(const shakti_params& p);

struct DevSell {
  int32_t n_rows = 0, n_cols = 0, n_slices = 0;
  int32_t max_width = 0;
  int64_t padded = 0, nnz = 0;
  DevBuf<int32_t> slice_ptr, col, rowlen;
  DevBuf<double> val;
  mutable DevBuf<float> valf;
  mutable DevBuf<__half> valh;
  void upload_pattern(const HostSell& h, int64_t nnz_);
  void refresh_f32(cudaStream_t s) const;
  void refresh_f16_scaled(const double* dinv, cudaStream_t s) const;
};

template <class T>
struct SellViewT {
  int32_t n_rows, n_slices;
  const int32_t* slice_ptr;
  const int32_t* col;
  const T* val;
};
using SellView = SellViewT<double>;
inline SellView view(const DevSell& a) { return {a.n_rows, a.n_slices, a.slice_ptr.p, a.col.p, a.val.p}; }
inline SellViewT<float> viewf(const DevSell& a) { return {a.n_rows, a.n_slices, a.slice_ptr.p, a.col.p, a.valf.p}; }
template <class T> inline SellViewT<T> view_as(const DevSell& a);
template <> inline SellViewT<double> view_as<double>(const DevSell& a) { return view(a); }
template <> inline SellViewT<float> view_as<float>(const DevSell& a) { return viewf(a); }

struct FieldPtrs {
  const double *x, *y, *h0, *N, *N_n, *b, *qx, *qy, *G, *melt, *storage, *inputs;
  const uint8_t* isbc;
};

void upload_k_rule(int n, const double* pts_xy, const double* wts, cudaStream_t s);
void upload_reaction_rule(int n, const double* pts_xy, const double* wts, cudaStream_t s);

void launch_kbar(int32_t ne, const int32_t* c0, const int32_t* c1, const int32_t* c2,
                 const double* x, const double* y, const double* b, const double* qx,
                 const double* qy, double* kbar, DevParams p, cudaStream_t s);
void launch_assemble_atomic(int32_t ne, int32_t n_owned, const int32_t* c0, const int32_t* c1,
                            const int32_t* c2, const int32_t* slot, FieldPtrs f, const double* kbar,
                            double dt, double N_bdry, double* F, double* Jval, int want_J,
                            DevParams p, cudaStream_t s);
struct AssemblyPlanView {
  int32_t n_owned, rows_per_block, n_blocks, cap, vcap;
  const int32_t *blk_eptr, *blk_elems;
  const uint16_t* blk_lv;
  const int32_t *blk_hptr, *blk_halo, *inc_ptr;
  const uint16_t* inc_code;
  const uint32_t* src;
};
void launch_assemble_blocks(const AssemblyPlanView& plan, FieldPtrs f, const double* kbar, double dt, double N_bdry,
                            const int32_t* slice_ptr, double* F, double* Jval, int want_J, DevParams p, cudaStream_t s);
void launch_apply_bc(int32_t n_owned, const uint8_t* isbc, const double* N, double N_bdry,
                     const int32_t* diag_pos, double* F, double* Jval, int want_J, cudaStream_t s);

enum {
  kDiagArea = 0, kDiagVolume, kDiagInput, kDiagMelt, kDiagClosure, kDiagStorage, kDiagOutflow, kDiagImbalance, kDiagIntN,
  kDiagSums,
  kDiagNegNmin = kDiagSums, kDiagNmax, kDiagBmax,
  kDiagVals
};
int diagnostics_parts(int32_t ne, int sm_count);
void launch_diagnostics(int32_t ne, const int32_t* c0, const int32_t* c1, const int32_t* c2, const uint8_t* counted, FieldPtrs f,
                        const double* kbar, double dt, DevParams p, int nparts, double* partial, double* vals, double* row,
                        double its, double residual, cudaStream_t s);
void launch_diagnostics_row(const double* vals, double* row, double dt, double its, double residual, cudaStream_t s);

void launch_update_q(int32_t n_owned, const int32_t* win, const double* x, const double* y,
                     const double* h0, const double* N, const double* b, double* qx, double* qy,
                     DevParams p, cudaStream_t s);
void launch_update_melt(int32_t n_owned, const int32_t* win, const double* x, const double* y,
                        const double* h0, const double* N, const double* b, const double* qx,
                        const double* qy, const double* G, const double* melt_old, double* melt_new,
                        DevParams p, cudaStream_t s);
void launch_update_q_melt(int32_t n_owned, const int32_t* win, const double* x, const double* y,
                          const double* h0, const double* N, const double* b, double* qx, double* qy,
                          const double* G, const double* melt_old, double* melt_new, DevParams p, cudaStream_t s);
void launch_update_b(int32_t n_owned, const int32_t* win, const double* x, const double* y,
                     const double* h0, const double* N, const double* b_old, const double* qx,
                     const double* qy, const double* G, const double* melt, double* b_new, double dt,
                     double b_min, DevParams p, cudaStream_t s);

template <class T> void launch_spmv(SellViewT<T> A, const T* x, T* y, cudaStream_t s);
template <class T> void launch_residual(SellViewT<T> A, const T* x, const T* b, T* r, cudaStream_t s);
template <class T> void launch_jacobi(SellViewT<T> A, const T* dinv, const T* b, const T* x, T* x_out, double omega, cudaStream_t s);
template <class T> void launch_spmv_add(SellViewT<T> A, const T* x, T* y, cudaStream_t s);
template <class T> void launch_scaled_mul(int64_t n, const T* a, const T* b, double scale, T* out, cudaStream_t s);
template <class T> void launch_fill_t(int64_t n, T v, T* x, cudaStream_t s);
void launch_d2f(int64_t n, const double* a, float* out, cudaStream_t s);
void launch_f2d(int64_t n, const float* a, double* out, cudaStream_t s);
void launch_extract_dinv(int32_t n, const int32_t* diag_pos, const double* val, double* dinv, cudaStream_t s);

struct Reducer {
  DevBuf<double> partial;
  DevBuf<unsigned int> counter;
  int max_blocks = 0;
  void init(int sm_count);
};
void launch_multi_dot(Reducer& red, int64_t n, int nvec, const double* V, int64_t ld, const double* w,
                      double* out, cudaStream_t s);
void launch_multi_axpy_neg(int64_t n, int nvec, const double* V, int64_t ld, const double* h, double* w,
                           cudaStream_t s);
bool launch_orth_update_dot(Reducer& red, int64_t n, int nvec, const double* V, int64_t ld, const double* h, double* w,
                            double* out, cudaStream_t s);
void launch_multi_axpy_neg_scale(int64_t n, int nvec, const double* V, int64_t ld, const double* h, double* w, double scale,
                                 cudaStream_t s);
void launch_combine(int64_t n, int nvec, const double* V, int64_t ld, const double* h, double* y,
                    cudaStream_t s);
void launch_readback(const double* src, double* dst_host, int count, cudaStream_t s);
void launch_axpy(int64_t n, double alpha, const double* x, double* y, cudaStream_t s);
void launch_xmy_masked(int64_t n, const double* a, const uint8_t* mask, double* out, cudaStream_t s);
void launch_gather(int64_t n, const int32_t* idx, const double* src, double* dst, cudaStream_t s);
void launch_scatter(int64_t n, const int32_t* idx, const double* src, double* dst, cudaStream_t s);
void launch_interp_grid(int64_t n, const double* px, const double* py, int nx, int ny, const double* xg, const double* yg,
                        const double* f, double* out, cudaStream_t s);
void launch_points_in_polygon(int64_t n, const double* px, const double* py, int m, const double* poly_xy, double* out,
                              cudaStream_t s);
void launch_head0(int64_t n, const double* z_b, const double* z_s, double ratio, double* h0, cudaStream_t s);
void launch_interleave(int64_t n, const double* a, const double* b, double* ab, cudaStream_t s);
void launch_deinterleave(int64_t n, const double* ab, double* a, double* b, cudaStream_t s);

}
```

shakti-fenics_b200/csrc/kernels.cu:

```cuda
#include <algorithm>
#include <cstdlib>
#include <ctime>

#include "device.h"

namespace shakti {

int64_t g_kernel_launches = 0;

bool pdl_enabled() {
  static const bool on = getenv("SHAKTI_PDL") == nullptr || atoi(getenv("SHAKTI_PDL")) != 0;
  return on;
}

static std::vector<std::pair<std::string, std::pair<double, int64_t>>> g_phases;
bool phase_trace_enabled() {
  static const bool on = getenv("SHAKTI_TRACE_PHASES") != nullptr;
  return on;
}
static double now_ms() {
  timespec ts;
  clock_gettime(CLOCK_MONOTONIC, &ts);
  return ts.tv_sec * 1e3 + ts.tv_nsec * 1e-6;
}
void phase_add(const char* name, double ms) {
  for (auto& p : g_phases)
    if (p.first == name) { p.second.first += ms; p.second.second++; return; }
  g_phases.push_back({name, {ms, 1}});
}
void phase_report(const char* title) {
  if (g_phases.empty()) return;
  fprintf(stderr, "[phases] %s:", title);
  for (auto& p : g_phases) fprintf(stderr, " %s=%.2fms/%lld", p.first.c_str(), p.second.first, (long long)p.second.second);
  fprintf(stderr, "\n");
  g_phases.clear();
}
PhaseScope::PhaseScope(const char* n, cudaStream_t st) : name(n), s(st), on(phase_trace_enabled()) {
  if (!on) return;
  cudaStreamSynchronize(s);
  t0 = now_ms();
}
PhaseScope::~PhaseScope() {
  if (!on) return;
  cudaStreamSynchronize(s);
  phase_add(name, now_ms() - t0);
}

DevParams make_dev_params(const shakti_params& p) {
  DevParams d;
  d.g = p.g; d.rho_i = p.rho_i; d.rho_w = p.rho_w; d.nu = p.nu; d.Lh = p.Lh;
  d.omega = p.omega; d.n = p.n; d.A = p.A;
  d.cm = 1.0 / p.rho_i - 1.0 / p.rho_w;
  d.rwg = p.rho_w * p.g;
  d.inv_rwg = 1.0 / d.rwg;
  d.inv_Lh = 1.0 / p.Lh;
  d.cm_over_Lh = d.cm / p.Lh;
  d.n_is_3 = (p.n == 3.0);
  return d;
}

void DevSell::upload_pattern(const HostSell& h, int64_t nnz_) {
  n_rows = (int32_t)h.n_rows; n_cols = (int32_t)h.n_cols; n_slices = (int32_t)h.n_slices;
  padded = h.padded(); nnz = nnz_;
  max_width = 0;
  for (int32_t l : h.rowlen) max_width = std::max(max_width, l);
  slice_ptr.upload(h.slice_ptr);
  col.upload(h.col);
  rowlen.upload(h.rowlen);
  val.alloc_zero(padded);
}

constexpr int kMaxQ = 64;
__constant__ double c_kq[4 * kMaxQ];
__constant__ int c_nkq;
__constant__ double c_rq[4 * kMaxQ];
__constant__ int c_nrq;

static void pack_rule(int n, const double* pts, const double* wts, double* out) {
  for (int k = 0; k < n; ++k) {
    out[4 * k + 0] = 1.0 - pts[2 * k] - pts[2 * k + 1];
    out[4 * k + 1] = pts[2 * k];
    out[4 * k + 2] = pts[2 * k + 1];
    out[4 * k + 3] = wts[k];
  }
}
void upload_k_rule(int n, const double* pts, const double* wts, cudaStream_t s) {
  SHAKTI_REQUIRE(n > 0 && n <= kMaxQ, "quadrature table must have 1..64 points");
  double h[4 * kMaxQ];
  pack_rule(n, pts, wts, h);
  SHAKTI_CUDA(cudaStreamSynchronize(s));
  SHAKTI_CUDA(cudaMemcpyToSymbol(c_kq, h, sizeof(double) * 4 * n));
  SHAKTI_CUDA(cudaMemcpyToSymbol(c_nkq, &n, sizeof(int)));
}
void upload_reaction_rule(int n, const double* pts, const double* wts, cudaStream_t s) {
  SHAKTI_REQUIRE(n > 0 && n <= kMaxQ, "quadrature table must have 1..64 points");
  double h[4 * kMaxQ];
  pack_rule(n, pts, wts, h);
  SHAKTI_CUDA(cudaStreamSynchronize(s));
  SHAKTI_CUDA(cudaMemcpyToSymbol(c_rq, h, sizeof(double) * 4 * n));
  SHAKTI_CUDA(cudaMemcpyToSymbol(c_nrq, &n, sizeof(int)));
}

struct Geo {
  double gx[3], gy[3];
  double detabs;
};

__device__ __forceinline__ Geo geometry(double x0, double y0, double x1, double y1, double x2, double y2) {
  Geo g;
  const double d1x = x1 - x0, d1y = y1 - y0, d2x = x2 - x0, d2y = y2 - y0;
  const double det = d1x * d2y - d2x * d1y;
  const double inv = 1.0 / det;
  g.gx[1] = d2y * inv;  g.gy[1] = -d2x * inv;
  g.gx[2] = -d1y * inv; g.gy[2] = d1x * inv;
  g.gx[0] = -g.gx[1] - g.gx[2];
  g.gy[0] = -g.gy[1] - g.gy[2];
  g.detabs = fabs(det);
  return g;
}

__device__ __forceinline__ double powabs(double a, double e, int e_is_2) {
  return e_is_2 ? a * a : pow(fabs(a), e);
}

__global__ void __launch_bounds__(256)
kbar_kernel(int32_t ne, const int32_t* __restrict__ c0, const int32_t* __restrict__ c1,
            const int32_t* __restrict__ c2, const double* __restrict__ x, const double* __restrict__ y,
            const double* __restrict__ b, const double* __restrict__ qx, const double* __restrict__ qy,
            double* __restrict__ kbar, DevParams p) {
  const int32_t e = blockIdx.x * blockDim.x + threadIdx.x;
  if (e >= ne) return;
  const int32_t v0 = c0[e], v1 = c1[e], v2 = c2[e];
  const double x0 = x[v0], y0 = y[v0], x1 = x[v1], y1 = y[v1], x2 = x[v2], y2 = y[v2];
  const double detabs = fabs((x1 - x0) * (y2 - y0) - (x2 - x0) * (y1 - y0));
  const double b0 = b[v0], b1 = b[v1], b2 = b[v2];
  const double qx0 = qx[v0], qx1 = qx[v1], qx2 = qx[v2];
  const double qy0 = qy[v0], qy1 = qy[v1], qy2 = qy[v2];
  const double cK = p.g / (12.0 * p.nu);
  const double cRe = p.omega / p.nu;
  double acc = 0.0;
  const int nq = c_nkq;
  for (int k = 0; k < nq; ++k) {
    const double l0 = c_kq[4 * k], l1 = c_kq[4 * k + 1], l2 = c_kq[4 * k + 2], w = c_kq[4 * k + 3];
    const double bq = fabs(l0 * b0 + l1 * b1 + l2 * b2);
    const double u = l0 * qx0 + l1 * qx1 + l2 * qx2;
    const double v = l0 * qy0 + l1 * qy1 + l2 * qy2;
    const double qn = sqrt(u * u + v * v);
    acc += w * (bq * bq * bq) * cK / (1.0 + cRe * qn);
  }
  kbar[e] = acc * detabs;
}

void launch_kbar(int32_t ne, const int32_t* c0, const int32_t* c1, const int32_t* c2, const double* x,
                 const double* y, const double* b, const double* qx, const double* qy, double* kbar,
                 DevParams p, cudaStream_t s) {
  if (ne == 0) return;
  SHAKTI_LAUNCH(kbar_kernel, div_up(ne, 256), 256, 0, s, ne, c0, c1, c2, x, y, b, qx, qy, kbar, p);
}

struct ElemOut {
  double F[3];
  double J[3][3];
};

template <bool ST>
__device__ __forceinline__ void reaction_radon7(double detabs, const double bb[3], const double Nv[3], const double Nn[3],
                                                const double st[3], double cs, double A, double& f0, double& f1, double& f2,
                                                double& m00, double& m01, double& m02, double& m11, double& m12, double& m22) {
  double dqv[3] = {0, 0, 0}, sv[3] = {0, 0, 0}, Sd = 0, Ss = 0;
  if (ST) {
#pragma unroll
    for (int i = 0; i < 3; ++i) { dqv[i] = Nv[i] - Nn[i]; sv[i] = st[i] * cs; }
    Sd = dqv[0] + dqv[1] + dqv[2];
    Ss = sv[0] + sv[1] + sv[2];
  }
  const double Sb = bb[0] + bb[1] + bb[2], SN = Nv[0] + Nv[1] + Nv[2];
  const double A3 = 3.0 * A;
  {
    const double w = 0.1125 * detabs, t = 1.0 / 3.0;
    const double bq = Sb * t, Nq = SN * t, N2 = Nq * Nq;
    double r = A * bq * Nq * N2, d = A3 * bq * N2;
    if (ST) {
      const double dq = Sd * t, sq = Ss * t;
      r += sq * dq;
      d += sq;
    }
    r *= w * t;
    d *= w * (t * t);
    f0 = f1 = f2 = r;
    m00 = m01 = m02 = m11 = m12 = m22 = d;
  }
  const double s15 = 3.872983346207417;
#pragma unroll
  for (int orb = 0; orb < 2; ++orb) {
    const double a = orb == 0 ? (6.0 - s15) / 21.0 : (6.0 + s15) / 21.0;
    const double w = (orb == 0 ? (155.0 - s15) : (155.0 + s15)) * (1.0 / 2400.0) * detabs;
    const double e = 1.0 - 3.0 * a;
    const double ab = a * Sb, aN = a * SN, ad = a * Sd, as = a * Ss;
    double r[3], d[3];
#pragma unroll
    for (int i = 0; i < 3; ++i) {
      const double bq = ab + e * bb[i], Nq = aN + e * Nv[i];
      const double N2 = Nq * Nq;
      double ri = A * bq * Nq * N2, di = A3 * bq * N2;
      if (ST) {
        const double dq = ad + e * dqv[i], sq = as + e * sv[i];
        ri += sq * dq;
        di += sq;
      }
      r[i] = w * ri;
      d[i] = w * di;
    }
    const double R = a * (r[0] + r[1] + r[2]), D = a * a * (d[0] + d[1] + d[2]);
    const double ae = a * e, ee = e * e;
    f0 += R + e * r[0]; f1 += R + e * r[1]; f2 += R + e * r[2];
    m00 += D + (2.0 * ae + ee) * d[0];
    m11 += D + (2.0 * ae + ee) * d[1];
    m22 += D + (2.0 * ae + ee) * d[2];
    m01 += D + ae * (d[0] + d[1]);
    m02 += D + ae * (d[0] + d[2]);
    m12 += D + ae * (d[1] + d[2]);
  }
}

__device__ __forceinline__ void element_core(const Geo& g, const double h[3], const double bb[3], const double mm[3],
                                             const double qxv[3], const double qyv[3], const double Nv[3],
                                             const double Nn[3], const double st[3], const double Gv[3],
                                             const double inp[3], double kb, double dt, const DevParams& p, ElemOut& o) {
  double ghx = 0, ghy = 0, gbx = 0, gby = 0, gmx = 0, gmy = 0;
#pragma unroll
  for (int i = 0; i < 3; ++i) {
    ghx += h[i] * g.gx[i];  ghy += h[i] * g.gy[i];
    gbx += bb[i] * g.gx[i]; gby += bb[i] * g.gy[i];
    gmx += mm[i] * g.gx[i]; gmy += mm[i] * g.gy[i];
  }
  const double gb2 = gbx * gbx + gby * gby;
  const double gmgb = gmx * gbx + gmy * gby;
  const double inv1 = 1.0 / (1.0 + gb2);
  double rl[3], rsum = 0, qxs = 0, qys = 0;
#pragma unroll
  for (int i = 0; i < 3; ++i) {
    const double m0 = (Gv[i] - p.rwg * (qxv[i] * ghx + qyv[i] * ghy)) * p.inv_Lh;
    const double md = (gb2 * mm[i] + bb[i] * gmgb) * inv1;
    rl[i] = p.cm * (m0 + md) - inp[i];
    rsum += rl[i];
    qxs += qxv[i];
    qys += qyv[i];
  }
  const double m24 = g.detabs * (1.0 / 24.0);
  const double kJ = -kb * p.inv_rwg;
  const double cadv = p.cm_over_Lh * m24;
#pragma unroll
  for (int a = 0; a < 3; ++a) {
    o.F[a] = kb * (ghx * g.gx[a] + ghy * g.gy[a]) + m24 * (rsum + rl[a]);
    const double qax = cadv * (qxs + qxv[a]), qay = cadv * (qys + qyv[a]);
#pragma unroll
    for (int b = 0; b < 3; ++b)
      o.J[a][b] = kJ * (g.gx[a] * g.gx[b] + g.gy[a] * g.gy[b]) + qax * g.gx[b] + qay * g.gy[b];
  }
  const double cs = p.inv_rwg / dt;
  double f0 = 0, f1 = 0, f2 = 0, m00 = 0, m01 = 0, m02 = 0, m11 = 0, m12 = 0, m22 = 0;
  if (p.n_is_3) {
    if (st[0] != 0.0 || st[1] != 0.0 || st[2] != 0.0)
      reaction_radon7<true>(g.detabs, bb, Nv, Nn, st, cs, p.A, f0, f1, f2, m00, m01, m02, m11, m12, m22);
    else
      reaction_radon7<false>(g.detabs, bb, Nv, Nn, st, cs, p.A, f0, f1, f2, m00, m01, m02, m11, m12, m22);
  } else {
    const double e1 = p.n - 1.0, e2 = p.n - 2.0;
    const int nq = c_nrq;
    for (int k = 0; k < nq; ++k) {
      const double l0 = c_rq[4 * k], l1 = c_rq[4 * k + 1], l2 = c_rq[4 * k + 2];
      const double w = c_rq[4 * k + 3] * g.detabs;
      const double bq = l0 * bb[0] + l1 * bb[1] + l2 * bb[2];
      const double Nq = l0 * Nv[0] + l1 * Nv[1] + l2 * Nv[2];
      const double dq = Nq - (l0 * Nn[0] + l1 * Nn[1] + l2 * Nn[2]);
      const double sq = (l0 * st[0] + l1 * st[1] + l2 * st[2]) * cs;
      const double sgn = Nq > 0 ? 1.0 : (Nq < 0 ? -1.0 : 0.0);
      const double p1 = pow(fabs(Nq), e1);
      const double clos = p.A * bq * Nq * p1;
      const double dclos = p.A * bq * (p1 + Nq * e1 * pow(fabs(Nq), e2) * sgn);
      const double r = w * (clos + sq * dq);
      const double d = w * (dclos + sq);
      f0 += r * l0; f1 += r * l1; f2 += r * l2;
      const double d0 = d * l0, d1 = d * l1;
      m00 += d0 * l0; m01 += d0 * l1; m02 += d0 * l2;
      m11 += d1 * l1; m12 += d1 * l2; m22 += d * l2 * l2;
    }
  }
  o.F[0] -= f0; o.F[1] -= f1; o.F[2] -= f2;
  o.J[0][0] -= m00; o.J[0][1] -= m01; o.J[0][2] -= m02;
  o.J[1][0] -= m01; o.J[1][1] -= m11; o.J[1][2] -= m12;
  o.J[2][0] -= m02; o.J[2][1] -= m12; o.J[2][2] -= m22;
}

__device__ __forceinline__ void element_FJ(const int32_t v[3], const FieldPtrs& f, double kb, double dt,
                                           const DevParams& p, ElemOut& o, double Nv[3]) {
  const Geo g = geometry(f.x[v[0]], f.y[v[0]], f.x[v[1]], f.y[v[1]], f.x[v[2]], f.y[v[2]]);
  double h[3], bb[3], mm[3], qxv[3], qyv[3], Nn[3], st[3], Gv[3], inp[3];
#pragma unroll
  for (int i = 0; i < 3; ++i) {
    Nv[i] = f.N[v[i]];
    h[i] = f.h0[v[i]] - Nv[i] * p.inv_rwg;
    bb[i] = f.b[v[i]];
    mm[i] = f.melt[v[i]];
    qxv[i] = f.qx[v[i]];
    qyv[i] = f.qy[v[i]];
    Nn[i] = f.N_n[v[i]];
    st[i] = f.storage[v[i]];
    Gv[i] = f.G[v[i]];
    inp[i] = f.inputs[v[i]];
  }
  element_core(g, h, bb, mm, qxv, qyv, Nv, Nn, st, Gv, inp, kb, dt, p, o);
}

__device__ __forceinline__ void apply_lifting(ElemOut& o, const double Nv[3], const bool bc[3], double N_bdry) {
#pragma unroll
  for (int b = 0; b < 3; ++b)
    if (bc[b]) {
      const double gx = N_bdry - Nv[b];
#pragma unroll
      for (int a = 0; a < 3; ++a) o.F[a] += o.J[a][b] * gx;
    }
}

__device__ __forceinline__ void element_FJ_staged(const int v[3], const double* __restrict__ sV, int vcap, double kb,
                                                  double dt, const DevParams& p, ElemOut& o, double Nv[3]) {
  const Geo g = geometry(sV[0 * vcap + v[0]], sV[1 * vcap + v[0]], sV[0 * vcap + v[1]], sV[1 * vcap + v[1]],
                         sV[0 * vcap + v[2]], sV[1 * vcap + v[2]]);
  double h[3], bb[3], mm[3], qxv[3], qyv[3], Nn[3], st[3];
#pragma unroll
  for (int i = 0; i < 3; ++i) {
    h[i] = sV[2 * vcap + v[i]];
    Nv[i] = sV[3 * vcap + v[i]];
    Nn[i] = sV[4 * vcap + v[i]];
    bb[i] = sV[5 * vcap + v[i]];
    qxv[i] = sV[6 * vcap + v[i]];
    qyv[i] = sV[7 * vcap + v[i]];
    mm[i] = sV[9 * vcap + v[i]];
    st[i] = sV[10 * vcap + v[i]];
  }
  double Gv[3], inp[3];
#pragma unroll
  for (int i = 0; i < 3; ++i) { Gv[i] = sV[8 * vcap + v[i]]; inp[i] = sV[11 * vcap + v[i]]; }
  element_core(g, h, bb, mm, qxv, qyv, Nv, Nn, st, Gv, inp, kb, dt, p, o);
}

__global__ void __launch_bounds__(128)
assemble_atomic_kernel(int32_t ne, int32_t n_owned, const int32_t* __restrict__ c0,
                       const int32_t* __restrict__ c1, const int32_t* __restrict__ c2,
                       const int32_t* __restrict__ slot, FieldPtrs f, const double* __restrict__ kbar,
                       double dt, double N_bdry, double* __restrict__ F, double* __restrict__ Jval,
                       int want_J, DevParams p) {
  const int32_t e = blockIdx.x * blockDim.x + threadIdx.x;
  if (e >= ne) return;
  const int32_t v[3] = {c0[e], c1[e], c2[e]};
  ElemOut o;
  double Nv[3];
  element_FJ(v, f, kbar[e], dt, p, o, Nv);
  const bool bc[3] = {f.isbc[v[0]] != 0, f.isbc[v[1]] != 0, f.isbc[v[2]] != 0};
  apply_lifting(o, Nv, bc, N_bdry);
#pragma unroll
  for (int a = 0; a < 3; ++a) {
    if (v[a] >= n_owned || bc[a]) continue;
    atomicAdd(&F[v[a]], o.F[a]);
    if (want_J) {
#pragma unroll
      for (int b = 0; b < 3; ++b)
        if (!bc[b]) atomicAdd(&Jval[slot[(size_t)(3 * a + b) * ne + e]], o.J[a][b]);
    }
  }
}

void launch_assemble_atomic(int32_t ne, int32_t n_owned, const int32_t* c0, const int32_t* c1,
                            const int32_t* c2, const int32_t* slot, FieldPtrs f, const double* kbar,
                            double dt, double N_bdry, double* F, double* Jval, int want_J, DevParams p,
                            cudaStream_t s) {
  if (ne == 0) return;
  SHAKTI_LAUNCH(assemble_atomic_kernel, div_up(ne, 128), 128, 0, s, ne, n_owned, c0, c1, c2, slot, f, kbar,
                dt, N_bdry, F, Jval, want_J, p);
}

enum { VX = 0, VY, VH, VN, VNN, VB, VQX, VQY, VG, VM, VS, VI, VFIELDS };

__global__ void __launch_bounds__(256, 2)
assemble_blocks_kernel(int32_t n_owned, int32_t rows_per_block, int32_t cap, int32_t vcap,
                       const int32_t* __restrict__ blk_eptr, const int32_t* __restrict__ blk_elems,
                       const uint16_t* __restrict__ blk_lv, const int32_t* __restrict__ blk_hptr,
                       const int32_t* __restrict__ blk_halo, const int32_t* __restrict__ inc_ptr,
                       const uint16_t* __restrict__ inc_code, const uint32_t* __restrict__ src, FieldPtrs f,
                       const double* __restrict__ kbar, double dt, double N_bdry, const int32_t* __restrict__ slice_ptr,
                       double* __restrict__ F, double* __restrict__ Jval, int want_J, DevParams p) {
  extern __shared__ double smem[];
  double* sV = smem;
  double* sK = smem + (size_t)VFIELDS * vcap;
  uint8_t* sBC = reinterpret_cast<uint8_t*>(sK + (size_t)12 * cap);
  const int32_t r0 = blockIdx.x * rows_per_block;
  const int32_t nrows = min(rows_per_block, n_owned - r0);
  const int32_t h0 = blk_hptr[blockIdx.x], nh = blk_hptr[blockIdx.x + 1] - h0;
  constexpr int kCellsPre = 4;
  const int32_t e0 = blk_eptr[blockIdx.x], e1 = blk_eptr[blockIdx.x + 1];
  double kb_pre[kCellsPre];
  uint32_t lv01_pre[kCellsPre], lv2_pre[kCellsPre];
#pragma unroll
  for (int c = 0; c < kCellsPre; ++c) {
    const int32_t le = threadIdx.x + c * blockDim.x;
    kb_pre[c] = 0.0; lv01_pre[c] = 0; lv2_pre[c] = 0;
    if (le < e1 - e0) {
      const uint16_t* lv = blk_lv + 3 * (size_t)(e0 + le);
      lv01_pre[c] = (uint32_t)lv[0] | ((uint32_t)lv[1] << 16);
      lv2_pre[c] = lv[2];
      kb_pre[c] = kbar[blk_elems[e0 + le]];
    }
  }
  for (int32_t i = threadIdx.x; i < nrows + nh; i += blockDim.x) {
    const int32_t g = i < nrows ? r0 + i : blk_halo[h0 + i - nrows];
    const double Ni = f.N[g];
    sV[VX * vcap + i] = f.x[g];
    sV[VY * vcap + i] = f.y[g];
    sV[VH * vcap + i] = f.h0[g] - Ni * p.inv_rwg;
    sV[VN * vcap + i] = Ni;
    sV[VNN * vcap + i] = f.N_n[g];
    sV[VB * vcap + i] = f.b[g];
    sV[VQX * vcap + i] = f.qx[g];
    sV[VQY * vcap + i] = f.qy[g];
    sV[VG * vcap + i] = f.G[g];
    sV[VM * vcap + i] = f.melt[g];
    sV[VS * vcap + i] = f.storage[g];
    sV[VI * vcap + i] = f.inputs[g];
    sBC[i] = f.isbc[g];
  }
  __syncthreads();
#pragma unroll 1
  for (int c = 0; c * (int32_t)blockDim.x + (int32_t)threadIdx.x < e1 - e0; ++c) {
    const int32_t le = threadIdx.x + c * blockDim.x;
    int v[3];
    double kb;
    if (c < kCellsPre) {
      uint32_t a01 = lv01_pre[0], a2 = lv2_pre[0];
      kb = kb_pre[0];
#pragma unroll
      for (int q = 1; q < kCellsPre; ++q)
        if (c == q) { a01 = lv01_pre[q]; a2 = lv2_pre[q]; kb = kb_pre[q]; }
      v[0] = a01 & 0xFFFFu; v[1] = a01 >> 16; v[2] = a2;
    } else {
      const uint16_t* lv = blk_lv + 3 * (size_t)(e0 + le);
      v[0] = lv[0]; v[1] = lv[1]; v[2] = lv[2];
      kb = kbar[blk_elems[e0 + le]];
    }
    ElemOut o;
    double Nv[3];
    element_FJ_staged(v, sV, vcap, kb, dt, p, o, Nv);
    const bool bc[3] = {sBC[v[0]] != 0, sBC[v[1]] != 0, sBC[v[2]] != 0};
    apply_lifting(o, Nv, bc, N_bdry);
#pragma unroll
    for (int a = 0; a < 3; ++a) {
      sK[a * cap + le] = o.F[a];
#pragma unroll
      for (int b = 0; b < 3; ++b) sK[(3 + 3 * a + b) * cap + le] = (bc[a] || bc[b]) ? 0.0 : o.J[a][b];
    }
  }
  constexpr int kPre = 8;
  const bool has_row = (int32_t)threadIdx.x < nrows;
  const int32_t row = r0 + threadIdx.x;
  int32_t base = 0, w = 0, ib = 0, ie = 0;
  uint32_t pre[kPre];
  if (has_row) {
    const int32_t slice = row >> 5;
    base = slice_ptr[slice];
    w = (slice_ptr[slice + 1] - base) >> 5;
    ib = inc_ptr[row];
    ie = inc_ptr[row + 1];
    if (want_J) {
#pragma unroll
      for (int k = 0; k < kPre; ++k) pre[k] = k < w ? src[base + 32 * k + (row & 31)] : 0xFFFFFFFFu;
    }
  }
  __syncthreads();
  if (!has_row) return;
  const bool rbc = sBC[threadIdx.x] != 0;
  double Fr = 0.0, Jd = 0.0;
  for (int32_t k = ib; k < ie; ++k) {
    const uint32_t code = inc_code[k];
    const uint32_t le = code >> 2, a = code & 3u;
    Fr += sK[a * cap + le];
    Jd += sK[(3 + 4 * a) * cap + le];
  }
  F[row] = rbc ? sV[VN * vcap + threadIdx.x] - N_bdry : Fr;
  if (!want_J) return;
  auto entry = [&](uint32_t s2, int32_t pos) {
    if (s2 == 0xFFFFFFFFu) return;
    double v;
    if (s2 == 0xFFFEFFFEu) v = rbc ? 1.0 : Jd;
    else {
      const uint32_t ca = s2 & 0xFFFFu, cb = s2 >> 16;
      v = sK[(3 + (ca & 15u)) * cap + (ca >> 4)];
      if (cb != 0xFFFFu) v += sK[(3 + (cb & 15u)) * cap + (cb >> 4)];
    }
    Jval[pos] = v;
  };
#pragma unroll
  for (int k = 0; k < kPre; ++k)
    if (k < w) entry(pre[k], base + 32 * k + (row & 31));
  for (int k = kPre; k < w; ++k) {
    const int32_t pos = base + 32 * k + (row & 31);
    entry(src[pos], pos);
  }
}

void launch_assemble_blocks(const AssemblyPlanView& pl, FieldPtrs f, const double* kbar, double dt, double N_bdry,
                            const int32_t* slice_ptr, double* F, double* Jval, int want_J, DevParams p, cudaStream_t s) {
  if (pl.n_blocks == 0) return;
  int dev = 0;
  SHAKTI_CUDA(cudaGetDevice(&dev));
  const size_t smem = ((size_t)VFIELDS * pl.vcap + (size_t)12 * pl.cap) * sizeof(double) + pl.vcap;
  static size_t configured[64] = {};
  if (smem > configured[dev & 63]) {
    SHAKTI_CUDA(cudaFuncSetAttribute(assemble_blocks_kernel, cudaFuncAttributeMaxDynamicSharedMemorySize, (int)smem));
    configured[dev & 63] = smem;
  }
  const int threads = pl.rows_per_block >= 256 ? 256 : 128;
  SHAKTI_LAUNCH(assemble_blocks_kernel, pl.n_blocks, threads, smem, s, pl.n_owned, pl.rows_per_block, pl.cap, pl.vcap,
                pl.blk_eptr, pl.blk_elems, pl.blk_lv, pl.blk_hptr, pl.blk_halo, pl.inc_ptr, pl.inc_code, pl.src, f, kbar, dt,
                N_bdry, slice_ptr, F, Jval, want_J, p);
}

__global__ void apply_bc_kernel(int32_t n_owned, const uint8_t* __restrict__ isbc, const double* __restrict__ N,
                                double N_bdry, const int32_t* __restrict__ diag_pos, double* __restrict__ F,
                                double* __restrict__ Jval, int want_J) {
  const int32_t i = blockIdx.x * blockDim.x + threadIdx.x;
  if (i >= n_owned || !isbc[i]) return;
  F[i] = N[i] - N_bdry;
  if (want_J) Jval[diag_pos[i]] = 1.0;
}
void launch_apply_bc(int32_t n_owned, const uint8_t* isbc, const double* N, double N_bdry,
                     const int32_t* diag_pos, double* F, double* Jval, int want_J, cudaStream_t s) {
  if (n_owned == 0) return;
  SHAKTI_LAUNCH(apply_bc_kernel, div_up(n_owned, 256), 256, 0, s, n_owned, isbc, N, N_bdry, diag_pos, F, Jval, want_J);
}

struct WinGeo {
  int32_t v[3];
  int loc;
  Geo g;
};
__device__ __forceinline__ WinGeo win_geometry(const int32_t* __restrict__ win, int32_t i,
                                               const double* __restrict__ x, const double* __restrict__ y) {
  WinGeo w;
  const int4 t = reinterpret_cast<const int4*>(win)[i];
  w.v[0] = t.x; w.v[1] = t.y; w.v[2] = t.z; w.loc = t.w;
  if (w.loc >= 0) w.g = geometry(x[t.x], y[t.x], x[t.y], y[t.y], x[t.z], y[t.z]);
  return w;
}
__device__ __forceinline__ void cell_grad(const WinGeo& w, const double f[3], double& gx, double& gy) {
  gx = f[0] * w.g.gx[0] + f[1] * w.g.gx[1] + f[2] * w.g.gx[2];
  gy = f[0] * w.g.gy[0] + f[1] * w.g.gy[1] + f[2] * w.g.gy[2];
}

__device__ __forceinline__ double melt_at_vertex(const WinGeo& w, int32_t i, const double* __restrict__ h0,
                                                 const double* __restrict__ N, const double* __restrict__ b,
                                                 const double* __restrict__ qx, const double* __restrict__ qy,
                                                 const double* __restrict__ G, const double* __restrict__ melt,
                                                 const DevParams& p) {
  double h[3], bb[3], mm[3];
#pragma unroll
  for (int a = 0; a < 3; ++a) {
    h[a] = h0[w.v[a]] - N[w.v[a]] / p.rwg;
    bb[a] = b[w.v[a]];
    mm[a] = melt[w.v[a]];
  }
  double ghx, ghy, gbx, gby, gmx, gmy;
  cell_grad(w, h, ghx, ghy);
  cell_grad(w, bb, gbx, gby);
  cell_grad(w, mm, gmx, gmy);
  const double gb2 = gbx * gbx + gby * gby;
  const double m0 = (G[i] - p.rwg * (qx[i] * ghx + qy[i] * ghy)) / p.Lh;
  const double md = (gb2 * melt[i] + b[i] * (gmx * gbx + gmy * gby)) / (1.0 + gb2);
  return m0 + md;
}

__global__ void __launch_bounds__(256)
update_b_kernel(int32_t n_owned, const int32_t* __restrict__ win, const double* __restrict__ x,
                const double* __restrict__ y, const double* __restrict__ h0, const double* __restrict__ N,
                const double* __restrict__ b_old, const double* __restrict__ qx, const double* __restrict__ qy,
                const double* __restrict__ G, const double* __restrict__ melt, double* __restrict__ b_new,
                double dt, double b_min, DevParams p) {
  const int32_t i = blockIdx.x * blockDim.x + threadIdx.x;
  if (i >= n_owned) return;
  const WinGeo w = win_geometry(win, i, x, y);
  double bn;
  if (w.loc < 0) bn = b_old[i];
  else {
    const double m = melt_at_vertex(w, i, h0, N, b_old, qx, qy, G, melt, p);
    const double Ni = N[i];
    const double clos = p.A * b_old[i] * Ni * powabs(Ni, p.n - 1.0, p.n_is_3);
    bn = b_old[i] + dt * (m / p.rho_i - clos);
  }
  b_new[i] = bn < b_min ? b_min : bn;
}
void launch_update_b(int32_t n_owned, const int32_t* win, const double* x, const double* y, const double* h0,
                     const double* N, const double* b_old, const double* qx, const double* qy, const double* G,
                     const double* melt, double* b_new, double dt, double b_min, DevParams p, cudaStream_t s) {
  if (n_owned == 0) return;
  SHAKTI_LAUNCH(update_b_kernel, div_up(n_owned, 256), 256, 0, s, n_owned, win, x, y, h0, N, b_old, qx, qy, G,
                melt, b_new, dt, b_min, p);
}

template <bool Q, bool MELT>
__global__ void __launch_bounds__(256)
update_q_melt_kernel(int32_t n_owned, const int32_t* __restrict__ win, const double* __restrict__ x,
                     const double* __restrict__ y, const double* __restrict__ h0, const double* __restrict__ N,
                     const double* __restrict__ b, double* __restrict__ qx, double* __restrict__ qy,
                     const double* __restrict__ G, const double* __restrict__ melt_old, double* __restrict__ melt_new,
                     DevParams p) {
  const int32_t i = blockIdx.x * blockDim.x + threadIdx.x;
  if (i >= n_owned) return;
  const WinGeo w = win_geometry(win, i, x, y);
  if (w.loc < 0) {
    if (MELT) melt_new[i] = melt_old[i];
    return;
  }
  double h[3], bb[3], mm[3] = {0.0, 0.0, 0.0};
#pragma unroll
  for (int a = 0; a < 3; ++a) {
    h[a] = h0[w.v[a]] - N[w.v[a]] / p.rwg;
    bb[a] = b[w.v[a]];
    if (MELT) mm[a] = melt_old[w.v[a]];
  }
  double ghx, ghy, gbx, gby, gmx, gmy;
  cell_grad(w, h, ghx, ghy);
  cell_grad(w, bb, gbx, gby);
  cell_grad(w, mm, gmx, gmy);
  const double b_i = w.loc == 0 ? bb[0] : (w.loc == 1 ? bb[1] : bb[2]);
  const double m_i = w.loc == 0 ? mm[0] : (w.loc == 1 ? mm[1] : mm[2]);
  double qxn = qx[i], qyn = qy[i];
  if (Q) {
    const double bi = fabs(b_i);
    const double Re = sqrt(qxn * qxn + qyn * qyn) / p.nu;
    const double p1 = -(bi * bi * bi) * p.g;
    const double p2 = 12.0 * p.nu * (1.0 + p.omega * Re);
    qxn = p1 * ghx / p2;
    qyn = p1 * ghy / p2;
    qx[i] = qxn;
    qy[i] = qyn;
  }
  if (!MELT) return;
  const double gb2 = gbx * gbx + gby * gby;
  const double m0 = (G[i] - p.rwg * (qxn * ghx + qyn * ghy)) / p.Lh;
  const double md = (gb2 * m_i + b_i * (gmx * gbx + gmy * gby)) / (1.0 + gb2);
  melt_new[i] = m0 + md;
}
void launch_update_q(int32_t n_owned, const int32_t* win, const double* x, const double* y, const double* h0,
                     const double* N, const double* b, double* qx, double* qy, DevParams p, cudaStream_t s) {
  if (n_owned == 0) return;
  SHAKTI_LAUNCH((update_q_melt_kernel<true, false>), div_up(n_owned, 256), 256, 0, s, n_owned, win, x, y, h0, N, b, qx, qy,
                nullptr, nullptr, nullptr, p);
}
void launch_update_melt(int32_t n_owned, const int32_t* win, const double* x, const double* y, const double* h0,
                        const double* N, const double* b, const double* qx, const double* qy, const double* G,
                        const double* melt_old, double* melt_new, DevParams p, cudaStream_t s) {
  if (n_owned == 0) return;
  SHAKTI_LAUNCH((update_q_melt_kernel<false, true>), div_up(n_owned, 256), 256, 0, s, n_owned, win, x, y, h0, N, b,
                const_cast<double*>(qx), const_cast<double*>(qy), G, melt_old, melt_new, p);
}
void launch_update_q_melt(int32_t n_owned, const int32_t* win, const double* x, const double* y, const double* h0,
                          const double* N, const double* b, double* qx, double* qy, const double* G,
                          const double* melt_old, double* melt_new, DevParams p, cudaStream_t s) {
  if (n_owned == 0) return;
  SHAKTI_LAUNCH((update_q_melt_kernel<true, true>), div_up(n_owned, 256), 256, 0, s, n_owned, win, x, y, h0, N, b, qx, qy,
                G, melt_old, melt_new, p);
}

enum { SPMV_SET = 0, SPMV_ADD = 1, SPMV_RESID = 2, SPMV_JACOBI = 3 };

template <class T, int KG>
__device__ __forceinline__ bool sell_row_dot(const SellViewT<T>& A, const T* __restrict__ x, int32_t& row, T& acc) {
  if (KG == 1) {
    row = blockIdx.x * blockDim.x + threadIdx.x;
    const int32_t slice = row >> 5;
    if (slice >= A.n_slices) return false;
    const int32_t base = A.slice_ptr[slice];
    const int32_t w = (A.slice_ptr[slice + 1] - base) >> 5;
    const int32_t* __restrict__ cp = A.col + base + (row & 31);
    const T* __restrict__ vp = A.val + base + (row & 31);
    acc = 0;
#pragma unroll 4
    for (int k = 0; k < w; ++k) acc += vp[32 * k] * x[cp[32 * k]];
    return row < A.n_rows;
  } else {
    __shared__ T psum[KG][32];
    const int32_t slice = blockIdx.x;
    const int lane = threadIdx.x & 31, g = threadIdx.x >> 5;
    row = slice * 32 + lane;
    const int32_t base = A.slice_ptr[slice];
    const int32_t w = (A.slice_ptr[slice + 1] - base) >> 5;
    const int32_t* __restrict__ cp = A.col + base + lane;
    const T* __restrict__ vp = A.val + base + lane;
    T a = 0;
    for (int k = g; k < w; k += KG) a += vp[32 * k] * x[cp[32 * k]];
    psum[g][lane] = a;
    __syncthreads();
    if (g != 0) return false;
#pragma unroll
    for (int j = 1; j < KG; ++j) a += psum[j][lane];
    acc = a;
    return row < A.n_rows;
  }
}
constexpr int32_t kWideRowsBelow = 300000;

template <int MODE, class T, int KG>
__global__ void __launch_bounds__(256)
spmv_sell_kernel(SellViewT<T> A, const T* __restrict__ x, const T* __restrict__ b, const T* __restrict__ dinv, T omega,
                 T* __restrict__ y) {
  pdl_sync();
  int32_t row;
  T acc;
  if (!sell_row_dot<T, KG>(A, x, row, acc)) return;
  if (MODE == SPMV_SET) y[row] = acc;
  else if (MODE == SPMV_ADD) y[row] += acc;
  else if (MODE == SPMV_RESID) y[row] = b[row] - acc;
  else y[row] = x[row] + omega * dinv[row] * (b[row] - acc);
}

template <int MODE, class T>
static void spmv_launch(SellViewT<T> A, const T* x, const T* b, const T* dinv, double omega, T* y, cudaStream_t s) {
  if (A.n_rows == 0) return;
  if (A.n_rows < kWideRowsBelow) {
    SHAKTI_LAUNCH_PDL((spmv_sell_kernel<MODE, T, 8>), A.n_slices, 256, 0, s, A, x, b, dinv, (T)omega, y);
    return;
  }
  const int64_t threads = (int64_t)A.n_slices * 32;
  SHAKTI_LAUNCH_PDL((spmv_sell_kernel<MODE, T, 1>), div_up(threads, 256), 256, 0, s, A, x, b, dinv, (T)omega, y);
}
template <class T> void launch_spmv(SellViewT<T> A, const T* x, T* y, cudaStream_t s) { spmv_launch<SPMV_SET, T>(A, x, nullptr, nullptr, 0, y, s); }
template <class T> void launch_spmv_add(SellViewT<T> A, const T* x, T* y, cudaStream_t s) { spmv_launch<SPMV_ADD, T>(A, x, nullptr, nullptr, 0, y, s); }
template <class T> void launch_residual(SellViewT<T> A, const T* x, const T* b, T* r, cudaStream_t s) { spmv_launch<SPMV_RESID, T>(A, x, b, nullptr, 0, r, s); }
template <class T> void launch_jacobi(SellViewT<T> A, const T* dinv, const T* b, const T* x, T* x_out, double omega, cudaStream_t s) {
  spmv_launch<SPMV_JACOBI, T>(A, x, b, dinv, omega, x_out, s);
}
#define SHAKTI_INSTANTIATE_SPMV(T)                                                                       \
  template void launch_spmv<T>(SellViewT<T>, const T*, T*, cudaStream_t);                                \
  template void launch_spmv_add<T>(SellViewT<T>, const T*, T*, cudaStream_t);                            \
  template void launch_residual<T>(SellViewT<T>, const T*, const T*, T*, cudaStream_t);                  \
  template void launch_jacobi<T>(SellViewT<T>, const T*, const T*, const T*, T*, double, cudaStream_t);
SHAKTI_INSTANTIATE_SPMV(double)
SHAKTI_INSTANTIATE_SPMV(float)

__global__ void d2f_kernel(int64_t n, const double* __restrict__ a, float* __restrict__ out) {
  const int64_t stride = (int64_t)gridDim.x * blockDim.x;
  for (int64_t i = (int64_t)blockIdx.x * blockDim.x + threadIdx.x; i < n; i += stride) out[i] = (float)a[i];
}
__global__ void f2d_kernel(int64_t n, const float* __restrict__ a, double* __restrict__ out) {
  const int64_t stride = (int64_t)gridDim.x * blockDim.x;
  for (int64_t i = (int64_t)blockIdx.x * blockDim.x + threadIdx.x; i < n; i += stride) out[i] = (double)a[i];
}
static int stream_blocks(int64_t n) { return (int)std::min<int64_t>(148 * 16, std::max<int64_t>(1, (n + 255) / 256)); }
void launch_d2f(int64_t n, const double* a, float* out, cudaStream_t s) {
  if (n == 0) return;
  SHAKTI_LAUNCH(d2f_kernel, stream_blocks(n), 256, 0, s, n, a, out);
}
void launch_f2d(int64_t n, const float* a, double* out, cudaStream_t s) {
  if (n == 0) return;
  SHAKTI_LAUNCH(f2d_kernel, stream_blocks(n), 256, 0, s, n, a, out);
}
__global__ void __launch_bounds__(256)
sell_scale_to_half_kernel(SellView A, const double* __restrict__ dinv, __half* __restrict__ out) {
  const int32_t row = blockIdx.x * blockDim.x + threadIdx.x;
  const int32_t slice = row >> 5;
  if (slice >= A.n_slices) return;
  const int32_t base = A.slice_ptr[slice] + (row & 31);
  const int32_t w = (A.slice_ptr[slice + 1] - A.slice_ptr[slice]) >> 5;
  const double s = row < A.n_rows ? dinv[row] : 0.0;
  for (int k = 0; k < w; ++k) out[base + 32 * k] = __float2half_rn((float)(s * A.val[base + 32 * k]));
}
void DevSell::refresh_f16_scaled(const double* dinv, cudaStream_t s) const {
  if (valh.n != (size_t)padded) valh.alloc((size_t)std::max<int64_t>(padded, 1));
  if (n_rows == 0) return;
  SHAKTI_LAUNCH(sell_scale_to_half_kernel, div_up((int64_t)n_slices * 32, 256), 256, 0, s, view(*this), dinv, valh.p);
}
void DevSell::refresh_f32(cudaStream_t s) const {
  if (valf.n != (size_t)padded) valf.alloc((size_t)padded);
  launch_d2f(padded, val.p, valf.p, s);
}
template <class T>
__global__ void scaled_mul_kernel(int64_t n, const T* __restrict__ a, const T* __restrict__ b, T scale, T* __restrict__ out) {
  pdl_sync();
  const int64_t stride = (int64_t)gridDim.x * blockDim.x;
  for (int64_t i = (int64_t)blockIdx.x * blockDim.x + threadIdx.x; i < n; i += stride) out[i] = scale * a[i] * b[i];
}
template <class T> void launch_scaled_mul(int64_t n, const T* a, const T* b, double scale, T* out, cudaStream_t s) {
  if (n == 0) return;
  SHAKTI_LAUNCH((scaled_mul_kernel<T>), stream_blocks(n), 256, 0, s, n, a, b, (T)scale, out);
}
template void launch_scaled_mul<double>(int64_t, const double*, const double*, double, double*, cudaStream_t);
template void launch_scaled_mul<float>(int64_t, const float*, const float*, double, float*, cudaStream_t);
template <class T>
__global__ void fill_t_kernel(int64_t n, T v, T* __restrict__ x) {
  pdl_sync();
  const int64_t stride = (int64_t)gridDim.x * blockDim.x;
  for (int64_t i = (int64_t)blockIdx.x * blockDim.x + threadIdx.x; i < n; i += stride) x[i] = v;
}
template <class T> void launch_fill_t(int64_t n, T v, T* x, cudaStream_t s) {
  if (n == 0) return;
  SHAKTI_LAUNCH((fill_t_kernel<T>), stream_blocks(n), 256, 0, s, n, v, x);
}
template void launch_fill_t<double>(int64_t, double, double*, cudaStream_t);
template void launch_fill_t<float>(int64_t, float, float*, cudaStream_t);

__global__ void extract_dinv_kernel(int32_t n, const int32_t* __restrict__ diag_pos, const double* __restrict__ val,
                                    double* __restrict__ dinv) {
  const int32_t i = blockIdx.x * blockDim.x + threadIdx.x;
  if (i >= n) return;
  const double d = val[diag_pos[i]];
  dinv[i] = d != 0.0 ? 1.0 / d : 1.0;
}
void launch_extract_dinv(int32_t n, const int32_t* diag_pos, const double* val, double* dinv, cudaStream_t s) {
  if (n == 0) return;
  SHAKTI_LAUNCH(extract_dinv_kernel, div_up(n, 256), 256, 0, s, n, diag_pos, val, dinv);
}

constexpr int kRedThreads = 256;

void Reducer::init(int sm_count) {
  max_blocks = sm_count * 8;
  partial.alloc((size_t)max_blocks * 32);
  counter.alloc_zero(1);
}

__device__ __forceinline__ double warp_sum(double v) {
#pragma unroll
  for (int o = 16; o > 0; o >>= 1) v += __shfl_xor_sync(0xffffffffu, v, o);
  return v;
}

template <int NV>
__global__ void __launch_bounds__(kRedThreads)
multi_dot_kernel(int64_t n, const double* __restrict__ V, int64_t ld, const double* __restrict__ w,
                 double* __restrict__ partial, unsigned int* __restrict__ counter, double* __restrict__ out) {
  double acc[NV];
#pragma unroll
  for (int k = 0; k < NV; ++k) acc[k] = 0.0;
  const int64_t stride = (int64_t)gridDim.x * blockDim.x;
  for (int64_t i = (int64_t)blockIdx.x * blockDim.x + threadIdx.x; i < n; i += stride) {
    const double wi = w[i];
#pragma unroll
    for (int k = 0; k < NV; ++k) acc[k] += V[k * ld + i] * wi;
  }
  __shared__ double sm[NV][kRedThreads / 32];
  __shared__ bool is_last;
  const int lane = threadIdx.x & 31, wid = threadIdx.x >> 5;
#pragma unroll
  for (int k = 0; k < NV; ++k) {
    const double v = warp_sum(acc[k]);
    if (lane == 0) sm[k][wid] = v;
  }
  __syncthreads();
  if (threadIdx.x < NV) {
    double v = 0.0;
#pragma unroll
    for (int j = 0; j < kRedThreads / 32; ++j) v += sm[threadIdx.x][j];
    partial[(size_t)blockIdx.x * NV + threadIdx.x] = v;
  }
  __threadfence();
  __syncthreads();
  if (threadIdx.x == 0) is_last = (atomicAdd(counter, 1u) == gridDim.x - 1);
  __syncthreads();
  if (!is_last) return;
  __threadfence();
  for (int k = wid; k < NV; k += kRedThreads / 32) {
    double v = 0.0;
    for (int b = lane; b < (int)gridDim.x; b += 32) v += partial[(size_t)b * NV + k];
    v = warp_sum(v);
    if (lane == 0) out[k] = v;
  }
  if (threadIdx.x == 0) *counter = 0u;
}

void launch_multi_dot(Reducer& red, int64_t n, int nvec, const double* V, int64_t ld, const double* w,
                      double* out, cudaStream_t s) {
  int blocks = (int)std::min<int64_t>(red.max_blocks, std::max<int64_t>(1, (n + kRedThreads * 4 - 1) / (kRedThreads * 4)));
  int done = 0;
  while (done < nvec) {
    const int c = std::min(8, nvec - done);
    const double* Vc = V + (int64_t)done * ld;
    double* oc = out + done;
    switch (c) {
      case 1: SHAKTI_LAUNCH(multi_dot_kernel<1>, blocks, kRedThreads, 0, s, n, Vc, ld, w, red.partial.p, red.counter.p, oc); break;
      case 2: SHAKTI_LAUNCH(multi_dot_kernel<2>, blocks, kRedThreads, 0, s, n, Vc, ld, w, red.partial.p, red.counter.p, oc); break;
      case 3: SHAKTI_LAUNCH(multi_dot_kernel<3>, blocks, kRedThreads, 0, s, n, Vc, ld, w, red.partial.p, red.counter.p, oc); break;
      case 4: SHAKTI_LAUNCH(multi_dot_kernel<4>, blocks, kRedThreads, 0, s, n, Vc, ld, w, red.partial.p, red.counter.p, oc); break;
      case 5: SHAKTI_LAUNCH(multi_dot_kernel<5>, blocks, kRedThreads, 0, s, n, Vc, ld, w, red.partial.p, red.counter.p, oc); break;
      case 6: SHAKTI_LAUNCH(multi_dot_kernel<6>, blocks, kRedThreads, 0, s, n, Vc, ld, w, red.partial.p, red.counter.p, oc); break;
      case 7: SHAKTI_LAUNCH(multi_dot_kernel<7>, blocks, kRedThreads, 0, s, n, Vc, ld, w, red.partial.p, red.counter.p, oc); break;
      default: SHAKTI_LAUNCH(multi_dot_kernel<8>, blocks, kRedThreads, 0, s, n, Vc, ld, w, red.partial.p, red.counter.p, oc); break;
    }
    done += c;
  }
}

template <int NV>
__global__ void __launch_bounds__(kRedThreads)
orth_update_dot_kernel(int64_t n, int nvec, const double* __restrict__ V, int64_t ld, const double* __restrict__ h,
                       double* __restrict__ w, double* __restrict__ partial, unsigned int* __restrict__ counter,
                       double* __restrict__ out) {
  double hk[NV], acc[NV + 1];
#pragma unroll
  for (int k = 0; k < NV; ++k) { hk[k] = k < nvec ? h[k] : 0.0; acc[k] = 0.0; }
  acc[NV] = 0.0;
  const int64_t stride = (int64_t)gridDim.x * blockDim.x;
  for (int64_t i = (int64_t)blockIdx.x * blockDim.x + threadIdx.x; i < n; i += stride) {
    double vk[NV];
    double a = 0.0;
#pragma unroll
    for (int k = 0; k < NV; ++k) {
      vk[k] = k < nvec ? V[k * ld + i] : 0.0;
      a += hk[k] * vk[k];
    }
    const double wn = w[i] - a;
    w[i] = wn;
#pragma unroll
    for (int k = 0; k < NV; ++k) acc[k] += vk[k] * wn;
    acc[NV] += wn * wn;
  }
  __shared__ double sm[NV + 1][kRedThreads / 32];
  __shared__ bool is_last;
  const int lane = threadIdx.x & 31, wid = threadIdx.x >> 5;
#pragma unroll
  for (int k = 0; k <= NV; ++k) {
    const double v = warp_sum(acc[k]);
    if (lane == 0) sm[k][wid] = v;
  }
  __syncthreads();
  if (threadIdx.x <= NV) {
    double v = 0.0;
#pragma unroll
    for (int j = 0; j < kRedThreads / 32; ++j) v += sm[threadIdx.x][j];
    partial[(size_t)blockIdx.x * (NV + 1) + threadIdx.x] = v;
  }
  __threadfence();
  __syncthreads();
  if (threadIdx.x == 0) is_last = (atomicAdd(counter, 1u) == gridDim.x - 1);
  __syncthreads();
  if (!is_last) return;
  __threadfence();
  for (int k = wid; k <= NV; k += kRedThreads / 32) {
    double v = 0.0;
    for (int b = lane; b < (int)gridDim.x; b += 32) v += partial[(size_t)b * (NV + 1) + k];
    v = warp_sum(v);
    if (lane == 0) {
      if (k < nvec) out[k] = v;
      else if (k == NV) out[nvec] = v;
    }
  }
  if (threadIdx.x == 0) *counter = 0u;
}

bool launch_orth_update_dot(Reducer& red, int64_t n, int nvec, const double* V, int64_t ld, const double* h, double* w,
                            double* out, cudaStream_t s) {
  if (nvec > 24) return false;
  const int blocks = (int)std::min<int64_t>(red.max_blocks, std::max<int64_t>(1, (n + kRedThreads * 4 - 1) / (kRedThreads * 4)));
  if (nvec <= 8) SHAKTI_LAUNCH(orth_update_dot_kernel<8>, blocks, kRedThreads, 0, s, n, nvec, V, ld, h, w, red.partial.p, red.counter.p, out);
  else if (nvec <= 16) SHAKTI_LAUNCH(orth_update_dot_kernel<16>, blocks, kRedThreads, 0, s, n, nvec, V, ld, h, w, red.partial.p, red.counter.p, out);
  else SHAKTI_LAUNCH(orth_update_dot_kernel<24>, blocks, kRedThreads, 0, s, n, nvec, V, ld, h, w, red.partial.p, red.counter.p, out);
  return true;
}

enum { COMB_SUB = 0, COMB_SET = 1, COMB_ADD = 2, COMB_SUB_SCALE = 3 };
template <int NV, int MODE>
__global__ void __launch_bounds__(256)
combine_kernel(int64_t n, const double* __restrict__ V, int64_t ld, const double* __restrict__ h,
               double* __restrict__ w, double scale) {
  double hk[NV];
#pragma unroll
  for (int k = 0; k < NV; ++k) hk[k] = h[k];
  const int64_t stride = (int64_t)gridDim.x * blockDim.x;
  for (int64_t i = (int64_t)blockIdx.x * blockDim.x + threadIdx.x; i < n; i += stride) {
    double acc = 0.0;
#pragma unroll
    for (int k = 0; k < NV; ++k) acc += hk[k] * V[k * ld + i];
    if (MODE == COMB_SUB) w[i] -= acc;
    else if (MODE == COMB_SET) w[i] = acc;
    else if (MODE == COMB_ADD) w[i] += acc;
    else w[i] = (w[i] - acc) * scale;
  }
}

template <int MODE>
static void combine_chunk(int c, int blocks, int64_t n, const double* V, int64_t ld, const double* h, double* w,
                          cudaStream_t s, double scale = 1.0) {
  switch (c) {
    case 1: SHAKTI_LAUNCH((combine_kernel<1, MODE>), blocks, 256, 0, s, n, V, ld, h, w, scale); break;
    case 2: SHAKTI_LAUNCH((combine_kernel<2, MODE>), blocks, 256, 0, s, n, V, ld, h, w, scale); break;
    case 3: SHAKTI_LAUNCH((combine_kernel<3, MODE>), blocks, 256, 0, s, n, V, ld, h, w, scale); break;
    case 4: SHAKTI_LAUNCH((combine_kernel<4, MODE>), blocks, 256, 0, s, n, V, ld, h, w, scale); break;
    case 5: SHAKTI_LAUNCH((combine_kernel<5, MODE>), blocks, 256, 0, s, n, V, ld, h, w, scale); break;
    case 6: SHAKTI_LAUNCH((combine_kernel<6, MODE>), blocks, 256, 0, s, n, V, ld, h, w, scale); break;
    case 7: SHAKTI_LAUNCH((combine_kernel<7, MODE>), blocks, 256, 0, s, n, V, ld, h, w, scale); break;
    default: SHAKTI_LAUNCH((combine_kernel<8, MODE>), blocks, 256, 0, s, n, V, ld, h, w, scale); break;
  }
}

void launch_multi_axpy_neg(int64_t n, int nvec, const double* V, int64_t ld, const double* h, double* w,
                           cudaStream_t s) {
  if (n == 0) return;
  for (int done = 0; done < nvec; done += 8)
    combine_chunk<COMB_SUB>(std::min(8, nvec - done), stream_blocks(n), n, V + (int64_t)done * ld, ld, h + done, w, s);
}
void launch_multi_axpy_neg_scale(int64_t n, int nvec, const double* V, int64_t ld, const double* h, double* w, double scale,
                                 cudaStream_t s) {
  if (n == 0) return;
  for (int done = 0; done < nvec; done += 8) {
    const int c = std::min(8, nvec - done);
    if (done + c >= nvec) combine_chunk<COMB_SUB_SCALE>(c, stream_blocks(n), n, V + (int64_t)done * ld, ld, h + done, w, s, scale);
    else combine_chunk<COMB_SUB>(c, stream_blocks(n), n, V + (int64_t)done * ld, ld, h + done, w, s);
  }
}
void launch_combine(int64_t n, int nvec, const double* V, int64_t ld, const double* h, double* y, cudaStream_t s) {
  if (n == 0) return;
  for (int done = 0; done < nvec; done += 8) {
    const int c = std::min(8, nvec - done);
    if (done == 0) combine_chunk<COMB_SET>(c, stream_blocks(n), n, V, ld, h, y, s);
    else combine_chunk<COMB_ADD>(c, stream_blocks(n), n, V + (int64_t)done * ld, ld, h + done, y, s);
  }
}

__global__ void readback_kernel(const double* __restrict__ src, double* __restrict__ dst_host, int count) {
  for (int i = threadIdx.x; i < count; i += blockDim.x) dst_host[i] = src[i];
  __threadfence_system();
}
void launch_readback(const double* src, double* dst_host, int count, cudaStream_t s) {
  if (count <= 0) return;
  SHAKTI_LAUNCH(readback_kernel, 1, 64, 0, s, src, dst_host, count);
}

__device__ __forceinline__ int grid_interval(const double* __restrict__ g, int n, double v) {
  int lo = 0, hi = n;
  while (lo < hi) {
    const int mid = (lo + hi) >> 1;
    if (g[mid] <= v) lo = mid + 1; else hi = mid;
  }
  return min(max(lo - 1, 0), n - 2);
}
__global__ void __launch_bounds__(256)
interp_grid_kernel(int64_t n, const double* __restrict__ px, const double* __restrict__ py, int nx, int ny,
                   const double* __restrict__ xg, const double* __restrict__ yg, const double* __restrict__ f,
                   double* __restrict__ out) {
  const int64_t i = (int64_t)blockIdx.x * blockDim.x + threadIdx.x;
  if (i >= n) return;
  const double x = px[i], y = py[i];
  const int ix = grid_interval(xg, nx, x), iy = grid_interval(yg, ny, y);
  const double tx = (x - xg[ix]) / (xg[ix + 1] - xg[ix]);
  const double ty = (y - yg[iy]) / (yg[iy + 1] - yg[iy]);
  const double f00 = f[(size_t)iy * nx + ix], f10 = f[(size_t)iy * nx + ix + 1];
  const double f01 = f[(size_t)(iy + 1) * nx + ix], f11 = f[(size_t)(iy + 1) * nx + ix + 1];
  out[i] = (1.0 - tx) * (1.0 - ty) * f00 + tx * (1.0 - ty) * f10 + (1.0 - tx) * ty * f01 + tx * ty * f11;
}
void launch_interp_grid(int64_t n, const double* px, const double* py, int nx, int ny, const double* xg, const double* yg,
                        const double* f, double* out, cudaStream_t s) {
  if (n == 0) return;
  SHAKTI_LAUNCH(interp_grid_kernel, div_up(n, 256), 256, 0, s, n, px, py, nx, ny, xg, yg, f, out);
}

__global__ void __launch_bounds__(256)
points_in_polygon_kernel(int64_t n, const double* __restrict__ px, const double* __restrict__ py, int m,
                         const double* __restrict__ poly, double* __restrict__ out) {
  __shared__ double sx[1025], sy[1025];
  const int64_t i = (int64_t)blockIdx.x * blockDim.x + threadIdx.x;
  const double x = i < n ? px[i] : 0.0, y = i < n ? py[i] : 0.0;
  bool inside = false;
  for (int base = 0; base < m; base += 1024) {
    const int cnt = min(1024, m - base);
    __syncthreads();
    for (int k = threadIdx.x; k <= cnt; k += blockDim.x) {
      const int v = (base + k) % m;
      sx[k] = poly[2 * v];
      sy[k] = poly[2 * v + 1];
    }
    __syncthreads();
    for (int k = 0; k < cnt; ++k) {
      const double x0 = sx[k], y0 = sy[k], x1 = sx[k + 1], y1 = sy[k + 1];
      if ((y0 > y) != (y1 > y)) {
        const double xc = x0 + (y - y0) * (x1 - x0) / (y1 - y0);
        if (x < xc) inside = !inside;
      }
    }
  }
  if (i < n) out[i] = inside ? 1.0 : 0.0;
}
void launch_points_in_polygon(int64_t n, const double* px, const double* py, int m, const double* poly, double* out,
                              cudaStream_t s) {
  if (n == 0) return;
  SHAKTI_LAUNCH(points_in_polygon_kernel, div_up(n, 256), 256, 0, s, n, px, py, m, poly, out);
}

__global__ void axpy_kernel(int64_t n, double alpha, const double* __restrict__ x, double* __restrict__ y) {
  const int64_t stride = (int64_t)gridDim.x * blockDim.x;
  for (int64_t i = (int64_t)blockIdx.x * blockDim.x + threadIdx.x; i < n; i += stride) y[i] += alpha * x[i];
}
void launch_axpy(int64_t n, double alpha, const double* x, double* y, cudaStream_t s) {
  if (n == 0) return;
  SHAKTI_LAUNCH(axpy_kernel, stream_blocks(n), 256, 0, s, n, alpha, x, y);
}
__global__ void xmy_masked_kernel(int64_t n, const double* __restrict__ a, const uint8_t* __restrict__ mask,
                                  double* __restrict__ out) {
  const int64_t stride = (int64_t)gridDim.x * blockDim.x;
  for (int64_t i = (int64_t)blockIdx.x * blockDim.x + threadIdx.x; i < n; i += stride) out[i] = mask[i] ? 0.0 : a[i];
}
void launch_xmy_masked(int64_t n, const double* a, const uint8_t* mask, double* out, cudaStream_t s) {
  if (n == 0) return;
  SHAKTI_LAUNCH(xmy_masked_kernel, stream_blocks(n), 256, 0, s, n, a, mask, out);
}
__global__ void gather_kernel(int64_t n, const int32_t* __restrict__ idx, const double* __restrict__ src,
                              double* __restrict__ dst) {
  const int64_t stride = (int64_t)gridDim.x * blockDim.x;
  for (int64_t i = (int64_t)blockIdx.x * blockDim.x + threadIdx.x; i < n; i += stride) dst[i] = src[idx[i]];
}
void launch_gather(int64_t n, const int32_t* idx, const double* src, double* dst, cudaStream_t s) {
  if (n == 0) return;
  SHAKTI_LAUNCH(gather_kernel, stream_blocks(n), 256, 0, s, n, idx, src, dst);
}
__global__ void scatter_kernel(int64_t n, const int32_t* __restrict__ idx, const double* __restrict__ src,
                               double* __restrict__ dst) {
  const int64_t stride = (int64_t)gridDim.x * blockDim.x;
  for (int64_t i = (int64_t)blockIdx.x * blockDim.x + threadIdx.x; i < n; i += stride) dst[idx[i]] = src[i];
}
void launch_scatter(int64_t n, const int32_t* idx, const double* src, double* dst, cudaStream_t s) {
  if (n == 0) return;
  SHAKTI_LAUNCH(scatter_kernel, stream_blocks(n), 256, 0, s, n, idx, src, dst);
}
__global__ void head0_kernel(int64_t n, const double* __restrict__ z_b, const double* __restrict__ z_s, double ratio,
                             double* __restrict__ h0) {
  const int64_t stride = (int64_t)gridDim.x * blockDim.x;
  for (int64_t i = (int64_t)blockIdx.x * blockDim.x + threadIdx.x; i < n; i += stride)
    h0[i] = z_b[i] + ratio * (z_s[i] - z_b[i]);
}
void launch_head0(int64_t n, const double* z_b, const double* z_s, double ratio, double* h0, cudaStream_t s) {
  if (n == 0) return;
  SHAKTI_LAUNCH(head0_kernel, stream_blocks(n), 256, 0, s, n, z_b, z_s, ratio, h0);
}
__global__ void interleave_kernel(int64_t n, const double* __restrict__ a, const double* __restrict__ b,
                                  double* __restrict__ ab) {
  const int64_t stride = (int64_t)gridDim.x * blockDim.x;
  for (int64_t i = (int64_t)blockIdx.x * blockDim.x + threadIdx.x; i < n; i += stride) {
    ab[2 * i] = a[i];
    ab[2 * i + 1] = b[i];
  }
}
void launch_interleave(int64_t n, const double* a, const double* b, double* ab, cudaStream_t s) {
  if (n == 0) return;
  SHAKTI_LAUNCH(interleave_kernel, stream_blocks(n), 256, 0, s, n, a, b, ab);
}
__global__ void deinterleave_kernel(int64_t n, const double* __restrict__ ab, double* __restrict__ a,
                                    double* __restrict__ b) {
  const int64_t stride = (int64_t)gridDim.x * blockDim.x;
  for (int64_t i = (int64_t)blockIdx.x * blockDim.x + threadIdx.x; i < n; i += stride) {
    a[i] = ab[2 * i];
    b[i] = ab[2 * i + 1];
  }
}
void launch_deinterleave(int64_t n, const double* ab, double* a, double* b, cudaStream_t s) {
  if (n == 0) return;
  SHAKTI_LAUNCH(deinterleave_kernel, stream_blocks(n), 256, 0, s, n, ab, a, b);
}

constexpr int kDiagThreads = 256;

__device__ __forceinline__ void diag_block_reduce(double (&v)[kDiagVals], double* __restrict__ sh, double* __restrict__ out) {
#pragma unroll
  for (int k = 0; k < kDiagVals; ++k) sh[k * kDiagThreads + threadIdx.x] = v[k];
  __syncthreads();
  for (int w = kDiagThreads / 2; w > 0; w >>= 1) {
    if ((int)threadIdx.x < w) {
#pragma unroll
      for (int k = 0; k < kDiagVals; ++k) {
        const double a = sh[k * kDiagThreads + threadIdx.x], b = sh[k * kDiagThreads + threadIdx.x + w];
        sh[k * kDiagThreads + threadIdx.x] = k < kDiagSums ? a + b : fmax(a, b);
      }
    }
    __syncthreads();
  }
  if (threadIdx.x < kDiagVals) out[threadIdx.x] = sh[threadIdx.x * kDiagThreads];
}

__global__ void __launch_bounds__(kDiagThreads)
diagnostics_kernel(int32_t ne, const int32_t* __restrict__ c0, const int32_t* __restrict__ c1, const int32_t* __restrict__ c2,
                   const uint8_t* __restrict__ counted, FieldPtrs f, const double* __restrict__ kbar, double dt, DevParams p,
                   double* __restrict__ partial) {
  __shared__ double sh[kDiagVals * kDiagThreads];
  double v[kDiagVals];
#pragma unroll
  for (int k = 0; k < kDiagVals; ++k) v[k] = k < kDiagSums ? 0.0 : -INFINITY;
  const int32_t stride = gridDim.x * blockDim.x;
  for (int32_t e = blockIdx.x * blockDim.x + threadIdx.x; e < ne; e += stride) {
    if (!counted[e]) continue;
    const int32_t vv[3] = {c0[e], c1[e], c2[e]};
    const Geo g = geometry(f.x[vv[0]], f.y[vv[0]], f.x[vv[1]], f.y[vv[1]], f.x[vv[2]], f.y[vv[2]]);
    double h[3], bb[3], mm[3], qxv[3], qyv[3], Nv[3], Nn[3], st[3], Gv[3], inp[3];
#pragma unroll
    for (int i = 0; i < 3; ++i) {
      Nv[i] = f.N[vv[i]];
      h[i] = f.h0[vv[i]] - Nv[i] * p.inv_rwg;
      bb[i] = f.b[vv[i]];
      mm[i] = f.melt[vv[i]];
      qxv[i] = f.qx[vv[i]];
      qyv[i] = f.qy[vv[i]];
      Nn[i] = f.N_n[vv[i]];
      st[i] = f.storage[vv[i]];
      Gv[i] = f.G[vv[i]];
      inp[i] = f.inputs[vv[i]];
    }
    ElemOut o;
    element_core(g, h, bb, mm, qxv, qyv, Nv, Nn, st, Gv, inp, kbar[e], dt, p, o);
#pragma unroll
    for (int a = 0; a < 3; ++a) {
      if (f.isbc[vv[a]]) v[kDiagOutflow] -= o.F[a];
      else v[kDiagImbalance] += o.F[a];
    }
    double ghx = 0, ghy = 0, gbx = 0, gby = 0, gmx = 0, gmy = 0;
#pragma unroll
    for (int i = 0; i < 3; ++i) {
      ghx += h[i] * g.gx[i];  ghy += h[i] * g.gy[i];
      gbx += bb[i] * g.gx[i]; gby += bb[i] * g.gy[i];
      gmx += mm[i] * g.gx[i]; gmy += mm[i] * g.gy[i];
    }
    const double gb2 = gbx * gbx + gby * gby, gmgb = gmx * gbx + gmy * gby, inv1 = 1.0 / (1.0 + gb2);
    double smelt = 0, sinp = 0, sb = 0, sN = 0, ss = 0, sd = 0, ssd = 0;
#pragma unroll
    for (int i = 0; i < 3; ++i) {
      smelt += (Gv[i] - p.rwg * (qxv[i] * ghx + qyv[i] * ghy)) * p.inv_Lh + (gb2 * mm[i] + bb[i] * gmgb) * inv1;
      sinp += inp[i];
      sb += bb[i];
      sN += Nv[i];
      const double d = Nv[i] - Nn[i];
      ss += st[i];
      sd += d;
      ssd += st[i] * d;
    }
    const double m6 = g.detabs * (1.0 / 6.0);
    v[kDiagArea] += 0.5 * g.detabs;
    v[kDiagVolume] += m6 * sb;
    v[kDiagInput] += m6 * sinp;
    v[kDiagMelt] += m6 * smelt;
    v[kDiagIntN] += m6 * sN;
    v[kDiagStorage] += p.inv_rwg / dt * g.detabs * (1.0 / 24.0) * (ss * sd + ssd);
    double clos = 0;
    if (p.n_is_3) {
      double f0, f1, f2, m00, m01, m02, m11, m12, m22;
      reaction_radon7<false>(g.detabs, bb, Nv, Nn, st, 0.0, p.A, f0, f1, f2, m00, m01, m02, m11, m12, m22);
      clos = f0 + f1 + f2;
    } else {
      const double e1 = p.n - 1.0;
      const int nq = c_nrq;
      for (int k = 0; k < nq; ++k) {
        const double l0 = c_rq[4 * k], l1 = c_rq[4 * k + 1], l2 = c_rq[4 * k + 2];
        const double bq = l0 * bb[0] + l1 * bb[1] + l2 * bb[2];
        const double Nq = l0 * Nv[0] + l1 * Nv[1] + l2 * Nv[2];
        clos += c_rq[4 * k + 3] * g.detabs * (p.A * bq * Nq * pow(fabs(Nq), e1));
      }
    }
    v[kDiagClosure] += clos;
#pragma unroll
    for (int i = 0; i < 3; ++i) {
      v[kDiagNegNmin] = fmax(v[kDiagNegNmin], -Nv[i]);
      v[kDiagNmax] = fmax(v[kDiagNmax], Nv[i]);
      v[kDiagBmax] = fmax(v[kDiagBmax], bb[i]);
    }
  }
  diag_block_reduce(v, sh, partial + (size_t)blockIdx.x * kDiagVals);
}

__device__ __forceinline__ void diag_write_row(const double* vals, double* row, double dt, double its, double residual) {
  row[SHAKTI_D_DT] = dt;
  row[SHAKTI_D_NEWTON_ITS] = its;
  row[SHAKTI_D_RESIDUAL] = residual;
#pragma unroll
  for (int k = 0; k <= kDiagImbalance; ++k) row[SHAKTI_D_AREA + k] = vals[k];
  row[SHAKTI_D_N_MEAN] = vals[kDiagIntN] / vals[kDiagArea];
  row[SHAKTI_D_N_MIN] = -vals[kDiagNegNmin];
  row[SHAKTI_D_N_MAX] = vals[kDiagNmax];
  row[SHAKTI_D_B_MAX] = vals[kDiagBmax];
}

__global__ void __launch_bounds__(kDiagThreads)
diagnostics_finish_kernel(int nparts, const double* __restrict__ partial, double* __restrict__ vals, double* __restrict__ row,
                          double dt, double its, double residual) {
  __shared__ double sh[kDiagVals * kDiagThreads];
  double v[kDiagVals];
#pragma unroll
  for (int k = 0; k < kDiagVals; ++k) v[k] = k < kDiagSums ? 0.0 : -INFINITY;
  for (int b = threadIdx.x; b < nparts; b += kDiagThreads)
#pragma unroll
    for (int k = 0; k < kDiagVals; ++k) v[k] = k < kDiagSums ? v[k] + partial[(size_t)b * kDiagVals + k] : fmax(v[k], partial[(size_t)b * kDiagVals + k]);
  diag_block_reduce(v, sh, vals);
  if (row == nullptr) return;
  __syncthreads();
  if (threadIdx.x == 0) diag_write_row(vals, row, dt, its, residual);
}

__global__ void diagnostics_row_kernel(const double* __restrict__ vals, double* __restrict__ row, double dt, double its,
                                       double residual) {
  diag_write_row(vals, row, dt, its, residual);
}

int diagnostics_parts(int32_t ne, int sm_count) { return std::max(1, std::min(div_up(ne, kDiagThreads), 4 * sm_count)); }

void launch_diagnostics(int32_t ne, const int32_t* c0, const int32_t* c1, const int32_t* c2, const uint8_t* counted, FieldPtrs f,
                        const double* kbar, double dt, DevParams p, int nparts, double* partial, double* vals, double* row,
                        double its, double residual, cudaStream_t s) {
  if (ne > 0) SHAKTI_LAUNCH(diagnostics_kernel, nparts, kDiagThreads, 0, s, ne, c0, c1, c2, counted, f, kbar, dt, p, partial);
  SHAKTI_LAUNCH(diagnostics_finish_kernel, 1, kDiagThreads, 0, s, ne > 0 ? nparts : 0, partial, vals, row, dt, its, residual);
}

void launch_diagnostics_row(const double* vals, double* row, double dt, double its, double residual, cudaStream_t s) {
  SHAKTI_LAUNCH(diagnostics_row_kernel, 1, 1, 0, s, vals, row, dt, its, residual);
}

}
```

Measured before the change: 9.774.

## Keep Chebyshev coefficients on device and fuse AMG cycle seams and fine refresh

Chebyshev bounds and coefficients are now computed on the device by a single-thread kernel, so the host readback and stream synchronize during refresh are gone and the CUDA graph no longer has to be invalidated on every refresh. The fine-level dinv, fp32 matrix copy and Gershgorin bound are fused into one grid-stride pass. The V-cycle seams are fused as well: the entry d2f is merged with the first Chebyshev step, restriction is merged with the coarse first step, and the last post-smooth writes z in double directly. In exchange there are more kernel variants and mode flags, a graph key check on matrix pointers, and coefficients read from device memory inside every smoothing kernel.

After: 10.18, median of 6. +4.1%, better.

```diff
diff --git a/shakti-fenics_b200/csrc/amg.cu b/shakti-fenics_b200/csrc/amg.cu
--- a/shakti-fenics_b200/csrc/amg.cu
+++ b/shakti-fenics_b200/csrc/amg.cu
@@ -370,10 +370,11 @@
   if (lane == 0) x[warp] = (TX)acc;
 }
 
-template <class T, int KG>
+enum { CHEBY_PLAIN = 0, CHEBY_X_IS_D = 1, CHEBY_EXIT = 2 };
+template <class T, int KG, int MODE = CHEBY_PLAIN>
 __global__ void __launch_bounds__(256)
 amg_cheby_kernel(SellViewT<T> A, const T* __restrict__ dinv, const T* __restrict__ b, const T* __restrict__ x,
-                 T* __restrict__ d, T* __restrict__ x_out, T c1, T c2) {
+                 T* __restrict__ d, T* __restrict__ x_out, const double* __restrict__ cf, double* __restrict__ z) {
   pdl_sync();
   int32_t row;
   T acc = 0;
@@ -404,24 +405,31 @@
     for (int j = 1; j < KG; ++j) acc += psum[j][lane];
   }
   if (row >= A.n_rows) return;
+  const T c1 = (T)cf[0], c2 = (T)cf[1];
   const T r = dinv[row] * (b[row] - acc);
-  const T dn = c1 * d[row] + c2 * r;
+  const T dn = c1 * (MODE == CHEBY_X_IS_D ? x[row] : d[row]) + c2 * r;
+  if (MODE == CHEBY_EXIT) {
+    z[row] = (double)(x[row] + dn);
+    return;
+  }
   d[row] = dn;
   x_out[row] = x[row] + dn;
 }
 constexpr int32_t kChebyWideRowsBelow = 300000;
-template <class T>
-static void launch_cheby(SellViewT<T> A, const T* dinv, const T* b, const T* x, T* d, T* x_out, double c1, double c2, cudaStream_t s) {
+template <class T, int MODE = CHEBY_PLAIN>
+static void launch_cheby(SellViewT<T> A, const T* dinv, const T* b, const T* x, T* d, T* x_out, const double* cf, cudaStream_t s) {
+  static_assert(MODE != CHEBY_EXIT, "the exit sweep writes z: launched by Amg::apply");
   if (A.n_rows < kChebyWideRowsBelow)
-    SHAKTI_LAUNCH_PDL((amg_cheby_kernel<T, 8>), A.n_slices, 256, 0, s, A, dinv, b, x, d, x_out, (T)c1, (T)c2);
+    SHAKTI_LAUNCH_PDL((amg_cheby_kernel<T, 8, MODE>), A.n_slices, 256, 0, s, A, dinv, b, x, d, x_out, cf, nullptr);
   else
-    SHAKTI_LAUNCH_PDL((amg_cheby_kernel<T, 1>), div_up((int64_t)A.n_slices * 32, 256), 256, 0, s, A, dinv, b, x, d, x_out, (T)c1, (T)c2);
+    SHAKTI_LAUNCH_PDL((amg_cheby_kernel<T, 1, MODE>), div_up((int64_t)A.n_slices * 32, 256), 256, 0, s, A, dinv, b, x, d, x_out, cf,
+                      nullptr);
 }
 
 __global__ void __launch_bounds__(256)
 amg_cheby_h_kernel(int32_t n_rows, int32_t n_slices, const int32_t* __restrict__ slice_ptr, const int32_t* __restrict__ col,
                    const __half* __restrict__ val, const float* __restrict__ dinv, const float* __restrict__ b,
-                   const float* __restrict__ x, float* __restrict__ d, float* __restrict__ x_out, float c1, float c2) {
+                   const float* __restrict__ x, float* __restrict__ d, float* __restrict__ x_out, const double* __restrict__ cf) {
   pdl_sync();
   const int32_t row = blockIdx.x * blockDim.x + threadIdx.x;
   const int32_t slice = row >> 5;
@@ -434,6 +442,7 @@
 #pragma unroll 4
   for (int k = 0; k < w; ++k) acc += __half2float(vp[32 * k]) * x[cp[32 * k]];
   if (row >= n_rows) return;
+  const float c1 = (float)cf[0], c2 = (float)cf[1];
   const float r = dinv[row] * b[row] - acc;
   const float dn = c1 * d[row] + c2 * r;
   d[row] = dn;
@@ -460,31 +469,103 @@
 }
 static bool uses_half(const Amg::Impl& I, const DevSell& A);
 
+__global__ void amg_cycle_entry_kernel(int32_t n, const double* __restrict__ r, const float* __restrict__ dinv,
+                                       const double* __restrict__ inv_theta, float* __restrict__ b, float* __restrict__ x) {
+  const int32_t i = blockIdx.x * blockDim.x + threadIdx.x;
+  if (i >= n) return;
+  const float bi = (float)r[i];
+  b[i] = bi;
+  x[i] = dinv[i] * bi * (float)inv_theta[0];
+}
+
 template <class T>
-__global__ void amg_cheby_first_kernel(int32_t n, const T* __restrict__ dinv, const T* __restrict__ b, T inv_theta,
-                                       T* __restrict__ d, T* __restrict__ x) {
+__global__ void amg_cheby_first_kernel(int32_t n, const T* __restrict__ dinv, const T* __restrict__ b,
+                                       const double* __restrict__ inv_theta, T* __restrict__ d, T* __restrict__ x) {
   pdl_sync();
   const int32_t i = blockIdx.x * blockDim.x + threadIdx.x;
   if (i >= n) return;
-  const T v = dinv[i] * b[i] * inv_theta;
+  const T v = dinv[i] * b[i] * (T)inv_theta[0];
   d[i] = v;
   x[i] = v;
 }
 
+__device__ __forceinline__ void block_max_to(double v, unsigned long long* __restrict__ out) {
+  __shared__ double wmax[8];
+#pragma unroll
+  for (int o = 16; o > 0; o >>= 1) v = fmax(v, __shfl_xor_sync(0xffffffffu, v, o));
+  if ((threadIdx.x & 31) == 0) wmax[threadIdx.x >> 5] = v;
+  __syncthreads();
+  if (threadIdx.x == 0) {
+#pragma unroll
+    for (int j = 1; j < 8; ++j) v = fmax(v, wmax[j]);
+    if (v > 0.0) atomicMax(out, (unsigned long long)__double_as_longlong(v));
+  }
+}
+static int bound_blocks(int64_t rows, int sm_count) { return (int)std::min<int64_t>((int64_t)sm_count * 8, std::max<int64_t>(1, div_up(rows, 256))); }
+
 __global__ void __launch_bounds__(256)
 amg_gershgorin_kernel(SellView A, const double* __restrict__ dinv, unsigned long long* __restrict__ out) {
-  const int32_t row = blockIdx.x * blockDim.x + threadIdx.x;
   double v = 0.0;
-  if (row < A.n_rows) {
+  for (int32_t row = blockIdx.x * blockDim.x + threadIdx.x; row < A.n_rows; row += gridDim.x * blockDim.x) {
     const int32_t base = A.slice_ptr[row >> 5] + (row & 31);
     const int32_t w = (A.slice_ptr[(row >> 5) + 1] - A.slice_ptr[row >> 5]) >> 5;
     double acc = 0.0;
     for (int k = 0; k < w; ++k) acc += fabs(A.val[base + 32 * k]);
-    v = fabs(dinv[row]) * acc;
-  }
-#pragma unroll
-  for (int o = 16; o > 0; o >>= 1) v = fmax(v, __shfl_xor_sync(0xffffffffu, v, o));
-  if ((threadIdx.x & 31) == 0 && v > 0.0) atomicMax(out, (unsigned long long)__double_as_longlong(v));
+    v = fmax(v, fabs(dinv[row]) * acc);
+  }
+  block_max_to(v, out);
+}
+
+template <bool F32>
+__global__ void __launch_bounds__(256)
+amg_fine_refresh_kernel(SellView A, const int32_t* __restrict__ diag_pos, double* __restrict__ dinv, float* __restrict__ dinvf,
+                        float* __restrict__ valf, unsigned long long* __restrict__ bound) {
+  double v = 0.0;
+  const int32_t rows = A.n_slices * 32;
+  for (int32_t row = blockIdx.x * blockDim.x + threadIdx.x; row < rows; row += gridDim.x * blockDim.x) {
+    const int32_t base = A.slice_ptr[row >> 5] + (row & 31);
+    const int32_t w = (A.slice_ptr[(row >> 5) + 1] - A.slice_ptr[row >> 5]) >> 5;
+    double di = 0.0;
+    if (row < A.n_rows) {
+      const double d = A.val[diag_pos[row]];
+      di = d != 0.0 ? 1.0 / d : 0.0;
+      dinv[row] = di;
+      dinvf[row] = (float)di;
+    }
+    double acc = 0.0;
+#pragma unroll 4
+    for (int k = 0; k < w; ++k) {
+      const double a = A.val[base + 32 * k];
+      if (F32) valf[base + 32 * k] = (float)a;
+      acc += fabs(a);
+    }
+    if (row < A.n_rows) v = fmax(v, fabs(di) * acc);
+  }
+  block_max_to(v, bound);
+}
+
+__global__ void amg_cheby_coef_kernel(int nl, int sweeps, int stride, double ratio, const double* __restrict__ bound, int keep,
+                                      double* __restrict__ lmax, double* __restrict__ coef) {
+  if (blockIdx.x != 0 || threadIdx.x != 0) return;
+  for (int l = 0; l < nl; ++l) {
+    const double h = bound[l];
+    if (h > 0.0 && isfinite(h)) lmax[l] = h;
+    else if (!keep) lmax[l] = 2.0;
+    const double hi = lmax[l], lo = __ddiv_rn(hi, ratio);
+    const double theta = __dmul_rn(0.5, __dadd_rn(hi, lo)), delta = __dmul_rn(0.5, __dsub_rn(hi, lo));
+    const double sigma = __ddiv_rn(theta, delta);
+    double rho = __ddiv_rn(1.0, sigma);
+    double* __restrict__ c = coef + (size_t)l * stride;
+    c[0] = __ddiv_rn(1.0, theta);
+    c[2] = 0.0;
+    c[3] = c[0];
+    for (int k = 1; k < sweeps; ++k) {
+      const double rho_n = __ddiv_rn(1.0, __dsub_rn(__dmul_rn(2.0, sigma), rho));
+      c[2 + 2 * k] = __dmul_rn(rho_n, rho);
+      c[3 + 2 * k] = __ddiv_rn(__dmul_rn(2.0, rho_n), delta);
+      rho = rho_n;
+    }
+  }
 }
 
 __global__ void amg_pack_rows_kernel(int64_t n, const int32_t* __restrict__ pos, const double* __restrict__ val,
@@ -560,7 +641,7 @@
   DevBuf<int32_t> tmap;
   CycleVecs<double> vd;
   CycleVecs<float> vf;
-  double lmax = 2.0;
+  int32_t index = 0;
   bool last = false;
   HostCsr hA;
   HostSell hS;
@@ -589,10 +670,14 @@
   bool built = false;
   double op_complexity = 0.0;
   Reducer red;
-  DevBuf<double> scal, lmax_dev;
-  double* host_scal = nullptr;
+  DevBuf<double> lmax_bound, lmax, coef;
+  int coef_stride = 0, coef_sweeps = 0;
+  DevBuf<double> fixed_coef;
   cudaGraphExec_t gexec = nullptr;
   bool graph_valid = false;
+  const void* graph_key[5] = {};
+  bool graph_seams = false;
+  const float* exit_x = nullptr;
   bool warm = false;
   int64_t graph_launches = 0;
   void* result_ptr = nullptr;
@@ -614,7 +699,6 @@
   P2pGather tail_gather;
   DevBuf<double> tail_rhs_d, tail_gather_d;
   ~Impl() {
-    if (host_scal) cudaFreeHost(host_scal);
     if (gexec) cudaGraphExecDestroy(gexec);
   }
 };
@@ -655,8 +739,7 @@
   I.sm_count = sm_count;
   I.tail.reset();
   I.tail_level = -1;
-  I.scal.alloc_zero(4, s);
-  if (!I.host_scal) SHAKTI_CUDA(cudaMallocHost(&I.host_scal, 32 * sizeof(double)));
+  I.fixed_coef.upload(std::vector<double>{0.3, 0.2});
   refreshes_ = 0;
 }
 
@@ -707,39 +790,66 @@
   return on && I.opt.fp32_cycle && I.opt.smoother == 1 && A.n_rows >= kChebyWideRowsBelow;
 }
 
-static void sync_cycle_precision(Amg::Impl& I, size_t l, const DevSell& Afine, bool matrices) {
+static void sync_cycle_precision(Amg::Impl& I, size_t l, const DevSell& Afine, bool matrices, bool fine_done = false) {
   cudaStream_t s = I.s;
   AmgLevel& L = *I.lv[l];
   const DevSell& A = (l == 0) ? Afine : L.A;
   if (I.opt.fp32_cycle) {
-    launch_d2f(L.n, L.dinv.p, L.vf.dinv.p, s);
-    if (uses_half(I, A)) A.refresh_f16_scaled(L.dinv.p, s);
-    else A.refresh_f32(s);
+    if (!(l == 0 && fine_done)) {
+      launch_d2f(L.n, L.dinv.p, L.vf.dinv.p, s);
+      if (uses_half(I, A)) A.refresh_f16_scaled(L.dinv.p, s);
+      else A.refresh_f32(s);
+    }
     if (matrices && !L.last) { L.P.refresh_f32(s); L.R.refresh_f32(s); }
   } else if (L.n) {
     SHAKTI_CUDA(cudaMemcpyAsync(L.vd.dinv.p, L.dinv.p, sizeof(double) * L.n, cudaMemcpyDeviceToDevice, s));
   }
 }
 
-static void update_smoother_bounds(Amg::Impl& I, const DevSell& Afine) {
+static bool fine_one_pass(const Amg::Impl& I) { return I.opt.fp32_cycle && I.opt.smoother == 1 && I.lv[0]->n > 0; }
+
+static void fine_refresh_pass(Amg::Impl& I, const DevSell& Afine, const int32_t* fine_diag_pos, double* bound) {
+  cudaStream_t s = I.s;
+  AmgLevel& L = *I.lv[0];
+  unsigned long long* b = reinterpret_cast<unsigned long long*>(bound);
+  const int grid = bound_blocks((int64_t)Afine.n_slices * 32, I.sm_count);
+  if (uses_half(I, Afine)) {
+    SHAKTI_LAUNCH(amg_fine_refresh_kernel<false>, grid, 256, 0, s, view(Afine), fine_diag_pos, L.dinv.p, L.vf.dinv.p, nullptr, b);
+    Afine.refresh_f16_scaled(L.dinv.p, s);
+  } else {
+    if (Afine.valf.n != (size_t)Afine.padded) Afine.valf.alloc((size_t)Afine.padded);
+    SHAKTI_LAUNCH(amg_fine_refresh_kernel<true>, grid, 256, 0, s, view(Afine), fine_diag_pos, L.dinv.p, L.vf.dinv.p, Afine.valf.p, b);
+  }
+}
+
+static void launch_cheby_coef(Amg::Impl& I, int nl, bool keep) {
+  SHAKTI_LAUNCH(amg_cheby_coef_kernel, 1, 32, 0, I.s, nl, I.coef_sweeps, I.coef_stride, I.opt.cheby_ratio, I.lmax_bound.p,
+                keep ? 1 : 0, I.lmax.p, I.coef.p);
+}
+
+static bool update_smoother_bounds(Amg::Impl& I, const DevSell& Afine, const int32_t* fine_diag_pos) {
   cudaStream_t s = I.s;
   const size_t nl = I.lv.size();
-  if (I.opt.smoother != 1) return;
-  if (I.lmax_dev.n < nl) { I.lmax_dev.alloc_zero(std::max<size_t>(nl, 16), s); }
-  SHAKTI_CUDA(cudaMemsetAsync(I.lmax_dev.p, 0, sizeof(double) * nl, s));
+  if (I.opt.smoother != 1) return false;
+  if (I.lmax_bound.n < nl) {
+    I.coef_sweeps = std::max({I.opt.presmooth, I.opt.postsmooth, 8});
+    I.coef_stride = 2 + 2 * I.coef_sweeps;
+    I.lmax_bound.alloc_zero(nl, s);
+    I.lmax.alloc_zero(nl, s);
+    I.coef.alloc_zero(nl * I.coef_stride, s);
+  }
+  SHAKTI_CUDA(cudaMemsetAsync(I.lmax_bound.p, 0, sizeof(double) * nl, s));
+  const bool fine = fine_one_pass(I);
   for (size_t l = 0; l < nl; ++l) {
     AmgLevel& L = *I.lv[l];
-    if (L.n > 0)
-      SHAKTI_LAUNCH(amg_gershgorin_kernel, div_up(L.n, 256), 256, 0, s, view(l == 0 ? Afine : L.A), L.dinv.p,
-                    reinterpret_cast<unsigned long long*>(I.lmax_dev.p + l));
-  }
-  comm_allreduce_max(I.lmax_dev.p, (int)nl, s);
-  std::vector<double> h(nl);
-  SHAKTI_REQUIRE(nl <= 32, "AMG: more than 32 levels");
-  launch_readback(I.lmax_dev.p, I.host_scal, (int)nl, s);
-  SHAKTI_CUDA(cudaStreamSynchronize(s));
-  for (size_t l = 0; l < nl; ++l) h[l] = I.host_scal[l];
-  for (size_t l = 0; l < nl; ++l) I.lv[l]->lmax = (h[l] > 0 && std::isfinite(h[l])) ? h[l] : 2.0;
+    if (l == 0 && fine) fine_refresh_pass(I, Afine, fine_diag_pos, I.lmax_bound.p);
+    else if (L.n > 0)
+      SHAKTI_LAUNCH(amg_gershgorin_kernel, bound_blocks(L.n, I.sm_count), 256, 0, s, view(l == 0 ? Afine : L.A), L.dinv.p,
+                    reinterpret_cast<unsigned long long*>(I.lmax_bound.p + l));
+  }
+  comm_allreduce_max(I.lmax_bound.p, (int)nl, s);
+  launch_cheby_coef(I, (int)nl, false);
+  return fine;
 }
 
 static void coarsen_level(Amg::Impl& I, size_t l, const DevSell& dA, const HostCsr& A, const HostSell& S,
@@ -928,6 +1038,7 @@
   Ln->hA = product_pattern(R, AP);
   Ln->hA.n_cols = (int64_t)nc + gc;
   Ln->hS = sell_from_csr(Ln->hA);
+  Ln->index = (int32_t)l + 1;
   Ln->n = nc;
   Ln->n_ghost = gc;
   Ln->n_cols = nc + gc;
@@ -1165,19 +1276,23 @@
   Impl& I = *p_;
   cudaStream_t s = I.s;
   if (!I.built || I.lv.empty()) return;
-  I.graph_valid = false;
   AmgLevel& L = *I.lv[0];
-  if (L.n > 0) SHAKTI_LAUNCH(amg_dinv_kernel, div_up(L.n, 256), 256, 0, s, L.n, fine_diag_pos, Afine.val.p, L.dinv.p);
-  if (I.opt.smoother != 1 || (L.last && I.dense_coarse)) { sync_cycle_precision(I, 0, Afine, false); return; }
-  SHAKTI_CUDA(cudaMemsetAsync(I.scal.p + 1, 0, sizeof(double), s));
-  if (L.n > 0)
-    SHAKTI_LAUNCH(amg_gershgorin_kernel, div_up(L.n, 256), 256, 0, s, view(Afine), L.dinv.p,
-                  reinterpret_cast<unsigned long long*>(I.scal.p + 1));
-  comm_allreduce_max(I.scal.p + 1, 1, s);
-  launch_readback(I.scal.p + 1, I.host_scal, 1, s);
-  SHAKTI_CUDA(cudaStreamSynchronize(s));
-  if (I.host_scal[0] > 0 && std::isfinite(I.host_scal[0])) L.lmax = I.host_scal[0];
-  sync_cycle_precision(I, 0, Afine, false);
+  const bool cheby = I.opt.smoother == 1 && !(L.last && I.dense_coarse);
+  if (cheby) SHAKTI_CUDA(cudaMemsetAsync(I.lmax_bound.p, 0, sizeof(double), s));
+  const bool fine = cheby && fine_one_pass(I);
+  if (fine) {
+    fine_refresh_pass(I, Afine, fine_diag_pos, I.lmax_bound.p);
+  } else {
+    if (L.n > 0) SHAKTI_LAUNCH(amg_dinv_kernel, div_up(L.n, 256), 256, 0, s, L.n, fine_diag_pos, Afine.val.p, L.dinv.p);
+    if (cheby && L.n > 0)
+      SHAKTI_LAUNCH(amg_gershgorin_kernel, bound_blocks(L.n, I.sm_count), 256, 0, s, view(Afine), L.dinv.p,
+                    reinterpret_cast<unsigned long long*>(I.lmax_bound.p));
+  }
+  if (cheby) {
+    comm_allreduce_max(I.lmax_bound.p, 1, s);
+    launch_cheby_coef(I, 1, true);
+  }
+  sync_cycle_precision(I, 0, Afine, false, fine);
 }
 
 void Amg::refresh(const DevSell& Afine, const int32_t* fine_diag_pos) {
@@ -1189,8 +1304,9 @@
     { SHAKTI_PHASE("rf_numeric", s); for (size_t l = 0; l < I.lv.size(); ++l) numeric_level(I, l, Afine, fine_diag_pos); }
     { SHAKTI_PHASE("rf_tail", s); refresh_tail(I, Afine); }
   }
-  { SHAKTI_PHASE("rf_bounds", s); update_smoother_bounds(I, Afine); }
-  { SHAKTI_PHASE("rf_f32", s); for (size_t l = 0; l < I.lv.size(); ++l) sync_cycle_precision(I, l, Afine, true); }
+  bool fine_done;
+  { SHAKTI_PHASE("rf_bounds", s); fine_done = update_smoother_bounds(I, Afine, fine_diag_pos); }
+  { SHAKTI_PHASE("rf_f32", s); for (size_t l = 0; l < I.lv.size(); ++l) sync_cycle_precision(I, l, Afine, true, fine_done); }
   if (I.dense_coarse) {
     AmgLevel& L = *I.lv.back();
     const DevSell& A = (I.lv.size() == 1) ? Afine : L.A;
@@ -1209,18 +1325,21 @@
 }
 
 template <class T>
-static void cheby_step(Amg::Impl& I, const DevSell& A, const T* dinv, const T* b, const T* x, T* d, T* x_out, double c1, double c2,
-                       cudaStream_t s) {
-  launch_cheby<T>(view_as<T>(A), dinv, b, x, d, x_out, c1, c2, s);
+static void cheby_step(Amg::Impl& I, const DevSell& A, const T* dinv, const T* b, const T* x, T* d, T* x_out, const double* cf,
+                       cudaStream_t s, bool x_is_d = false) {
+  if (x_is_d) launch_cheby<T, CHEBY_X_IS_D>(view_as<T>(A), dinv, b, x, d, x_out, cf, s);
+  else launch_cheby<T>(view_as<T>(A), dinv, b, x, d, x_out, cf, s);
 }
 template <>
 void cheby_step<float>(Amg::Impl& I, const DevSell& A, const float* dinv, const float* b, const float* x, float* d, float* x_out,
-                       double c1, double c2, cudaStream_t s) {
-  if (uses_half(I, A))
+                       const double* cf, cudaStream_t s, bool x_is_d) {
+  if (x_is_d)
+    launch_cheby<float, CHEBY_X_IS_D>(viewf(A), dinv, b, x, d, x_out, cf, s);
+  else if (uses_half(I, A))
     SHAKTI_LAUNCH_PDL(amg_cheby_h_kernel, div_up((int64_t)A.n_slices * 32, 256), 256, 0, s, A.n_rows, A.n_slices, A.slice_ptr.p, A.col.p,
-                      A.valh.p, dinv, b, x, d, x_out, (float)c1, (float)c2);
+                      A.valh.p, dinv, b, x, d, x_out, cf);
   else
-    launch_cheby<float>(viewf(A), dinv, b, x, d, x_out, c1, c2, s);
+    launch_cheby<float>(viewf(A), dinv, b, x, d, x_out, cf, s);
 }
 template <class T>
 static void level_residual(Amg::Impl& I, const DevSell& A, const T* dinv, const T* x, const T* b, T* r, cudaStream_t s) {
@@ -1235,8 +1354,10 @@
     launch_residual<float>(viewf(A), x, b, r, s);
 }
 
+enum { kSeamEntry = 1, kSeamExit = 2 };
 template <class T>
-static void smooth(Amg::Impl& I, AmgLevel& L, const DevSell& A, const T* b, int sweeps, bool zero_guess, bool ghosts_current) {
+static void smooth(Amg::Impl& I, AmgLevel& L, const DevSell& A, const T* b, int sweeps, bool zero_guess, bool ghosts_current,
+                   int seam = 0) {
   cudaStream_t s = I.s;
   CycleVecs<T>& v = vecs<T>(L);
   if (sweeps <= 0) {
@@ -1244,25 +1365,21 @@
     return;
   }
   if (I.opt.smoother == 1) {
-    const double hi = L.lmax, lo = L.lmax / I.opt.cheby_ratio;
-    const double theta = 0.5 * (hi + lo), delta = 0.5 * (hi - lo), sigma = theta / delta;
-    double rho = 1.0 / sigma;
+    SHAKTI_REQUIRE(sweeps <= I.coef_sweeps, "AMG: more Chebyshev sweeps than coefficients");
+    const double* cf = I.coef.p + (size_t)L.index * I.coef_stride;
     int k0 = 0;
     if (zero_guess) {
-      if (L.n) SHAKTI_LAUNCH_PDL((amg_cheby_first_kernel<T>), div_up(L.n, 256), 256, 0, s, L.n, v.dinv.p, b, (T)(1.0 / theta), v.d.p, v.x.p);
+      if (L.n && !(seam & kSeamEntry))
+        SHAKTI_LAUNCH_PDL((amg_cheby_first_kernel<T>), div_up(L.n, 256), 256, 0, s, L.n, v.dinv.p, b, cf, v.d.p, v.x.p);
       k0 = 1;
     }
     for (int k = k0; k < sweeps; ++k) {
-      double c1, c2;
-      if (k == 0) { c1 = 0.0; c2 = 1.0 / theta; }
-      else {
-        const double rho_n = 1.0 / (2.0 * sigma - rho);
-        c1 = rho_n * rho;
-        c2 = 2.0 * rho_n / delta;
-        rho = rho_n;
-      }
       if (I.opt.smoother_halo && !(ghosts_current && k == k0)) L.halo->exchange(v.x.p, s);
-      if (L.n) cheby_step<T>(I, A, v.dinv.p, b, v.x.p, v.d.p, v.x2.p, c1, c2, s);
+      if ((seam & kSeamExit) && k == sweeps - 1) {
+        I.exit_x = reinterpret_cast<const float*>(v.x.p);
+        break;
+      }
+      if (L.n) cheby_step<T>(I, A, v.dinv.p, b, v.x.p, v.d.p, v.x2.p, cf + 2 + 2 * k, s, (seam & kSeamEntry) && k == k0);
       std::swap(v.x.p, v.x2.p);
     }
   } else {
@@ -1277,8 +1394,13 @@
   }
 }
 
+static bool restrict_starts(const Amg::Impl& I, size_t c) {
+  const AmgLevel& C = *I.lv[c];
+  return I.opt.smoother == 1 && I.opt.presmooth >= 2 && !C.last && (int)c != I.tail_level && !uses_half(I, C.A);
+}
+
 template <class T>
-static void vcycle(Amg::Impl& I, const DevSell& Afine) {
+static void vcycle(Amg::Impl& I, const DevSell& Afine, bool seams) {
   cudaStream_t s = I.s;
   const int nl = (int)I.lv.size();
   for (int l = 0; l < nl; ++l) {
@@ -1322,10 +1444,15 @@
       }
       break;
     }
-    smooth<T>(I, L, A, v.b.p, I.opt.presmooth, true, false);
+    const bool started = l > 0 && restrict_starts(I, l);
+    smooth<T>(I, L, A, v.b.p, I.opt.presmooth, true, false, (seams && l == 0) || started ? kSeamEntry : 0);
     L.halo->exchange(v.x.p, s);
     level_residual<T>(I, A, v.dinv.p, v.x.p, v.b.p, v.r.p, s);
-    launch_spmv<T>(view_as<T>(L.R), v.r.p, vecs<T>(*I.lv[l + 1]).b.p, s);
+    CycleVecs<T>& vc = vecs<T>(*I.lv[l + 1]);
+    if (restrict_starts(I, l + 1))
+      launch_restrict_cheby_first<T>(view_as<T>(L.R), v.r.p, vc.dinv.p, I.coef.p + (size_t)(l + 1) * I.coef_stride, vc.b.p, vc.x.p, s);
+    else
+      launch_spmv<T>(view_as<T>(L.R), v.r.p, vc.b.p, s);
   }
   for (int l = nl - 2; l >= 0; --l) {
     AmgLevel& L = *I.lv[l];
@@ -1334,12 +1461,12 @@
     AmgLevel& C = *I.lv[l + 1];
     if (l + 1 != I.tail_level) C.halo->exchange(vecs<T>(C).x.p, s);
     launch_spmv_add<T>(view_as<T>(L.P), vecs<T>(C).x.p, v.x.p, s);
-    smooth<T>(I, L, A, v.b.p, I.opt.postsmooth, false, true);
+    smooth<T>(I, L, A, v.b.p, I.opt.postsmooth, false, true, seams && l == 0 ? kSeamExit : 0);
   }
 }
 
 template <class T>
-static void run_cycle(Amg::Impl& I, const DevSell& Afine) {
+static void run_cycle(Amg::Impl& I, const DevSell& Afine, bool seams = false) {
   cudaStream_t s = I.s;
   std::vector<std::pair<T*, T*>> saved;
   for (auto& L : I.lv) saved.push_back({vecs<T>(*L).x.p, vecs<T>(*L).x2.p});
@@ -1348,17 +1475,21 @@
     for (size_t l = 0; l < I.lv.size(); ++l) { vecs<T>(*I.lv[l]).x.p = saved[l].first; vecs<T>(*I.lv[l]).x2.p = saved[l].second; }
   };
   if (!I.opt.cuda_graph || !I.warm) {
-    vcycle<T>(I, Afine);
+    vcycle<T>(I, Afine, seams);
     restore();
     I.warm = true;
     return;
   }
+  const void* key[5] = {Afine.slice_ptr.p, Afine.col.p, Afine.val.p, Afine.valf.p, Afine.valh.p};
+  if (!std::equal(key, key + 5, I.graph_key) || seams != I.graph_seams) I.graph_valid = false;
   if (!I.graph_valid) {
+    std::copy(key, key + 5, I.graph_key);
+    I.graph_seams = seams;
     const int64_t before = g_kernel_launches;
     SHAKTI_CUDA(cudaStreamBeginCapture(s, cudaStreamCaptureModeRelaxed));
     cudaGraph_t graph = nullptr;
     try {
-      vcycle<T>(I, Afine);
+      vcycle<T>(I, Afine, seams);
     } catch (...) {
       cudaStreamEndCapture(s, &graph);
       if (graph) cudaGraphDestroy(graph);
@@ -1392,8 +1523,8 @@
   if (nnz) *nnz = A.nnz;
   if (value_bytes) *value_bytes = uses_half(I, A) ? 2 : (I.opt.fp32_cycle ? 4 : 8);
   if (L.n == 0) return true;
-  if (I.opt.fp32_cycle) cheby_step<float>(I, A, L.vf.dinv.p, L.vf.b.p, L.vf.x.p, L.vf.d.p, L.vf.x2.p, 0.3, 0.2, I.s);
-  else launch_cheby<double>(view(A), L.vd.dinv.p, L.vd.b.p, L.vd.x.p, L.vd.d.p, L.vd.x2.p, 0.3, 0.2, I.s);
+  if (I.opt.fp32_cycle) cheby_step<float>(I, A, L.vf.dinv.p, L.vf.b.p, L.vf.x.p, L.vf.d.p, L.vf.x2.p, I.fixed_coef.p, I.s);
+  else launch_cheby<double>(view(A), L.vd.dinv.p, L.vd.b.p, L.vd.x.p, L.vd.d.p, L.vd.x2.p, I.fixed_coef.p, I.s);
   return true;
 }
 
@@ -1407,11 +1538,28 @@
 template const float* Amg::cycle<float>(const DevSell&);
 template const double* Amg::cycle<double>(const DevSell&);
 
+static bool seams_apply(const Amg::Impl& I, const DevSell& Afine) {
+  const AmgLevel& L0 = *I.lv[0];
+  return I.opt.fp32_cycle && I.opt.smoother == 1 && I.opt.presmooth >= 2 && I.opt.postsmooth >= 1 && !L0.last &&
+         I.tail_level != 0 && L0.n > 0 && !uses_half(I, Afine);
+}
+
 void Amg::apply(const DevSell& Afine, const double* rin, double* z) {
   Impl& I = *p_;
   cudaStream_t s = I.s;
   AmgLevel& L0 = *I.lv[0];
-  if (I.opt.fp32_cycle) {
+  if (seams_apply(I, Afine)) {
+    SHAKTI_LAUNCH(amg_cycle_entry_kernel, div_up(L0.n, 256), 256, 0, s, L0.n, rin, L0.vf.dinv.p, I.coef.p, L0.vf.b.p, L0.vf.x.p);
+    run_cycle<float>(I, Afine, true);
+    const double* cf = I.coef.p + 2 + 2 * (I.opt.postsmooth - 1);
+    const SellViewT<float> A = viewf(Afine);
+    if (A.n_rows < kChebyWideRowsBelow)
+      SHAKTI_LAUNCH((amg_cheby_kernel<float, 8, CHEBY_EXIT>), A.n_slices, 256, 0, s, A, L0.vf.dinv.p, L0.vf.b.p, I.exit_x, L0.vf.d.p,
+                    nullptr, cf, z);
+    else
+      SHAKTI_LAUNCH((amg_cheby_kernel<float, 1, CHEBY_EXIT>), div_up((int64_t)A.n_slices * 32, 256), 256, 0, s, A, L0.vf.dinv.p,
+                    L0.vf.b.p, I.exit_x, L0.vf.d.p, nullptr, cf, z);
+  } else if (I.opt.fp32_cycle) {
     launch_d2f(L0.n, rin, L0.vf.b.p, s);
     run_cycle<float>(I, Afine);
     launch_f2d(L0.n, static_cast<const float*>(I.result_ptr), z, s);
diff --git a/shakti-fenics_b200/csrc/device.h b/shakti-fenics_b200/csrc/device.h
--- a/shakti-fenics_b200/csrc/device.h
+++ b/shakti-fenics_b200/csrc/device.h
@@ -102,6 +102,8 @@
 template <class T> void launch_residual(SellViewT<T> A, const T* x, const T* b, T* r, cudaStream_t s);
 template <class T> void launch_jacobi(SellViewT<T> A, const T* dinv, const T* b, const T* x, T* x_out, double omega, cudaStream_t s);
 template <class T> void launch_spmv_add(SellViewT<T> A, const T* x, T* y, cudaStream_t s);
+template <class T>
+void launch_restrict_cheby_first(SellViewT<T> R, const T* r, const T* dinv_c, const double* inv_theta, T* b_c, T* x_c, cudaStream_t s);
 template <class T> void launch_scaled_mul(int64_t n, const T* a, const T* b, double scale, T* out, cudaStream_t s);
 template <class T> void launch_fill_t(int64_t n, T v, T* x, cudaStream_t s);
 void launch_d2f(int64_t n, const double* a, float* out, cudaStream_t s);
diff --git a/shakti-fenics_b200/csrc/kernels.cu b/shakti-fenics_b200/csrc/kernels.cu
--- a/shakti-fenics_b200/csrc/kernels.cu
+++ b/shakti-fenics_b200/csrc/kernels.cu
@@ -732,6 +732,31 @@
   const int64_t threads = (int64_t)A.n_slices * 32;
   SHAKTI_LAUNCH_PDL((spmv_sell_kernel<MODE, T, 1>), div_up(threads, 256), 256, 0, s, A, x, b, dinv, (T)omega, y);
 }
+template <class T, int KG>
+__global__ void __launch_bounds__(256)
+restrict_cheby_first_kernel(SellViewT<T> R, const T* __restrict__ r, const T* __restrict__ dinv_c,
+                            const double* __restrict__ inv_theta, T* __restrict__ b_c, T* __restrict__ x_c) {
+  pdl_sync();
+  int32_t row;
+  T acc;
+  if (!sell_row_dot<T, KG>(R, r, row, acc)) return;
+  b_c[row] = acc;
+  x_c[row] = dinv_c[row] * acc * (T)inv_theta[0];
+}
+template <class T>
+void launch_restrict_cheby_first(SellViewT<T> R, const T* r, const T* dinv_c, const double* inv_theta, T* b_c, T* x_c, cudaStream_t s) {
+  if (R.n_rows == 0) return;
+  if (R.n_rows < kWideRowsBelow)
+    SHAKTI_LAUNCH_PDL((restrict_cheby_first_kernel<T, 8>), R.n_slices, 256, 0, s, R, r, dinv_c, inv_theta, b_c, x_c);
+  else
+    SHAKTI_LAUNCH_PDL((restrict_cheby_first_kernel<T, 1>), div_up((int64_t)R.n_slices * 32, 256), 256, 0, s, R, r, dinv_c, inv_theta,
+                      b_c, x_c);
+}
+template void launch_restrict_cheby_first<double>(SellViewT<double>, const double*, const double*, const double*, double*, double*,
+                                                  cudaStream_t);
+template void launch_restrict_cheby_first<float>(SellViewT<float>, const float*, const float*, const double*, float*, float*,
+                                                 cudaStream_t);
+
 template <class T> void launch_spmv(SellViewT<T> A, const T* x, T* y, cudaStream_t s) { spmv_launch<SPMV_SET, T>(A, x, nullptr, nullptr, 0, y, s); }
 template <class T> void launch_spmv_add(SellViewT<T> A, const T* x, T* y, cudaStream_t s) { spmv_launch<SPMV_ADD, T>(A, x, nullptr, nullptr, 0, y, s); }
 template <class T> void launch_residual(SellViewT<T> A, const T* x, const T* b, T* r, cudaStream_t s) { spmv_launch<SPMV_RESID, T>(A, x, b, nullptr, 0, r, s); }
```
